# ieellee/uLLSAM

Measured on AMD Instinct MI355X. Metric: images/s end-to-end (ViT+LLM+mask) 1024^2, higher is better.
Workload: dtype bf16; 1 GPU; uLLSAM mask path (app.py:580-645): SAM ViT-H + InternLM2-7b-shaped prefill S=1081 + prompt encoder + mask decoder + x4 upsample/threshold, 1 point prompt/image, batch 4/GPU; batch_per_gpu=4, global_batch=4, seq_len=1081, vit_linears=bf16

## Files before the change

### include/ullsam_hip.h

```cpp
#ifndef ULLSAM_HIP_H
#define ULLSAM_HIP_H
#ifdef __cplusplus
extern "C" {
#endif

#define ULLSAM_DT_F32 0
#define ULLSAM_DT_BF16 1
#define ULLSAM_ACT_NONE 0
#define ULLSAM_ACT_GELU 1
#define ULLSAM_ACT_RELU 2
#define ULLSAM_ACT_SWIGLU 3

#define ULLSAM_ABI_VERSION 14

const char* ullsam_last_error_string(void);
int ullsam_abi_version(void);
int ullsam_device_count(void);
int ullsam_set_gemm_variant(int variant);
int ullsam_set_gemm_tuning(int key, int value);
int ullsam_set_attn_variant(int variant);
int ullsam_set_attn_debug(void* stamps);

#define ULLSAM_ACT_SPLITK_OK 256
int ullsam_gemm(int dtype, const void* A, long lda, const void* W, long ldw, void* C, long ldc, int out_f32,
                const float* bias, const float* residual, long ldr, int res_row_mod, int act, int M, int N, int K,
                void* workspace, long ws_bytes, void* stream);

int ullsam_gemm_qkv_rope(int dtype, const void* A, long lda, const void* W, long ldw, const float* bias, int B, int S, int K, int KVH,
                         int G, const int* pos, const float* cos_tab, const float* sin_tab, int tab_rows, void* q_out, void* k_cache,
                         void* v_cache, int cap, int cache_pos0, void* workspace, long ws_bytes, void* stream);

int ullsam_gemm_panels(int dtype, const void* A, long lda, const void* W, long ldw, const void* w_panels, void* C, long ldc, int out_f32,
                       const float* bias, const float* residual, long ldr, int res_row_mod, int act, int M, int N, int K,
                       void* workspace, long ws_bytes, void* stream);
int ullsam_gemm_qkv_rope_panels(int dtype, const void* A, long lda, const void* W, long ldw, const void* w_panels, const float* bias, int B, int S,
                                int K, int KVH, int G, const int* pos, const float* cos_tab, const float* sin_tab, int tab_rows, void* q_out,
                                void* k_cache, void* v_cache, int cap, int cache_pos0, void* workspace, long ws_bytes, void* stream);

int ullsam_gemm_act_panels(int dtype, const void* A, long lda, const void* W, long ldw, const void* w_panels, void* C, long ldc, int out_f32,
                           const float* bias, const float* residual, long ldr, int res_row_mod, int act, int M, int N, int K,
                           void* workspace, long ws_bytes, int a_panels, int out_panels, void* stream);
int ullsam_gemm_qkv_rope_act_panels(int dtype, const void* A, long lda, const void* W, long ldw, const void* w_panels, const float* bias, int B, int S,
                                    int K, int KVH, int G, const int* pos, const float* cos_tab, const float* sin_tab, int tab_rows, void* q_out,
                                    void* k_cache, void* v_cache, int cap, int cache_pos0, void* workspace, long ws_bytes, int a_panels, void* stream);
int ullsam_gemm_act_panels_query(int dtype, int M, int N, int K, int act, int out_f32, int has_bias, int has_residual, int aligned, long ws_bytes,
                                 int* reads_a_panels, int* writes_c_panels);

int ullsam_gemm_rmsnorm(const float* x, long ldx, const float* norm_w, float eps, const void* W, long ldw, void* C, long ldc, int out_f32,
                        const float* bias, const float* residual, long ldr, int act, int M, int N, int K, void* stream);
int ullsam_decode_qkv_rope(const void* a, const float* x, long ldx, const float* norm_w, float eps, const void* W, long ldw, const float* bias,
                           int B, int K, int KVH, int G, const int* pos, const float* cos_tab, const float* sin_tab, int tab_rows, void* q_out,
                           void* k_cache, void* v_cache, int cap, int cache_pos0, void* stream);

int ullsam_train_matmul(const float* A, const float* B, float* C, int M, int N, int K, int batch, long a_b, long a_m, long a_k, long b_b,
                        long b_k, long b_n, long c_b, long c_m, long c_n, int accumulate, void* stream);
int ullsam_train_matmul_bf16(const float* A, const float* B, float* C, int M, int N, int K, int batch, long a_b, long a_m, long a_k, long b_b,
                             long b_k, long b_n, long c_b, long c_m, long c_n, int accumulate, void* stream);
int ullsam_train_matmul_heads(const float* A, const float* B, float* C, int M, int N, int K, int outer, int heads, long a_o, long a_h, int a_hdiv, long a_m, long a_k,
                              long b_o, long b_h, int b_hdiv, long b_k, long b_n, long c_o, long c_h, long c_m, long c_n, int accumulate, int bf16, int tri, void* stream);
int ullsam_train_matmul_splitk(const float* A, const float* B, float* C, int M, int N, int K, int batch, long a_b, long a_m, long a_k, long b_b,
                               long b_k, long b_n, long c_b, long c_m, long c_n, int accumulate, int ksplit, float* partial, void* stream);
int ullsam_train_set_matmul_mfma(int on);
int ullsam_train_set_matmul_vec(int on);
int ullsam_train_colsum(const float* x, float* out, long rows, int cols, long ld, float* partial, void* stream);
int ullsam_train_ln_bwd(const float* x, const float* w, const float* dy, float* dx, float* dw, float* db, long rows, int D, float eps, float* ws, void* stream);
int ullsam_train_act(const float* x, const float* dy, float* out, long n, int kind, void* stream);
int ullsam_train_scale_shift(const float* x, const float* s, const float* t, const float* dy, float* out, float* ds, float* dt, long n, float* partial, void* stream);
int ullsam_train_attention(const float* q, const float* k, const float* v, const float* dout, float* out, float* dq, float* dk, float* dv,
                           int B, int H, int groups, int hd, int Sq, int Sk, int causal, const int* key_mask, long q_bs, long q_ts, long q_hs,
                           long k_bs, long k_ts, long k_hs, long v_bs, long v_ts, long v_hs, long o_bs, long o_ts, long o_hs, float scale,
                           const float* bias_h, const float* bias_w, float* dbias_h, float* dbias_w, int kw, void* stream);
int ullsam_train_col2im3x3(const float* dcols, float* dx, int B, int H, int W, int C, void* stream);
int ullsam_train_attn_rows(float* S, float* dP, const float* bias_h, const float* bias_w, float* dbias_h, float* dbias_w, const int* key_mask,
                           int B, int H, int Sq, int Sk, int kw, int causal, int have_p, void* stream);
int ullsam_train_set_rows_reg(int on);
int ullsam_train_rmsnorm_bwd(const float* x, const float* w, const float* dy, float* dx, float* dw_rows, long rows, int D, float eps, void* stream);
int ullsam_train_rope(const float* x, const int* pos, const float* cos_tab, const float* sin_tab, float* out, long tokens, int heads, int hd,
                      int tab_rows, int adjoint, void* stream);
int ullsam_train_swiglu(const float* g, const float* u, const float* dy, float* out, float* dg, float* du, long n, void* stream);
int ullsam_train_resize_bwd(const float* dout, float* din, long planes, int ih, int iw, int oh, int ow, void* stream);
int ullsam_train_seg_loss(const float* x, const float* t, float* sums, float* losses, int P, long npix, float smooth, float* partial, void* stream);
int ullsam_train_seg_loss_bwd(const float* x, const float* t, const float* sums, const float* gscale, float* dx, int P, long npix, float smooth, void* stream);
int ullsam_train_cross_entropy(const float* logits, long ld, const long long* labels, float* lse, float* loss_rows, float* out2, long rows, int V, void* stream);
int ullsam_train_cross_entropy_bwd(const float* logits, long ld, const long long* labels, const float* lse, const float* out2, const float* gscale, float* dlogits,
                                   long ldx, long rows, int V, void* stream);
int ullsam_train_cross_entropy_bwd_bf16(const float* logits, long ld, const long long* labels, const float* lse, const float* out2, const float* gscale,
                                        void* dlog, long ldd, void* dlogT, long ldt, long rows, int V, void* stream);
int ullsam_train_embedding_bwd(const float* dx, long ldx, const int* sorted_ids, const int* order, const int* skip, long rows, int D, int V, int padding_idx,
                               void* table_grad, int out_dtype, void* stream);
int ullsam_train_index_add_rows(const float* src, const int* idx, float* dst, long rows, int C, int nrows_dst, void* stream);

int ullsam_norm(const void* in, int in_dtype, long in_stride, void* out, int out_dtype, long out_stride, const float* w,
                const float* b, long rows, int D, float eps, int rms, int act, const float* post_scale,
                const float* post_shift, void* stream);
int ullsam_norm_panels(const void* in, int in_dtype, long in_stride, void* out, const float* w, const float* b, long rows, int D, float eps, int rms,
                       int act, const float* post_scale, const float* post_shift, int out_panels, void* stream);
int ullsam_set_norm_variant(int v);

int ullsam_norm_fanout(const float* in, long rows, int D, const float* w, const float* b, float eps, float* out_f32, void* out_c,
                       void* out_c_pe, int c_dtype, const float* pe, long pe_rows, void* stream);

int ullsam_vit_attention(int dtype, const void* qkv, void* out, const void* rel_h, const void* rel_w, const void* qkv_bias,
                         int B, int heads, int hd, int grid_h, int grid_w, int window, void* stream);

int ullsam_causal_attention(int dtype, const void* q, const void* k, const void* v, void* out, const int* key_mask, int B,
                            int H, int KVH, int hd, int Sq, int Sk, int k_cap, int q_pos0, void* stream);

int ullsam_naive_attention(int dtype, const void* q, const void* k, const void* v, void* out, const int* key_mask, int B,
                           int H, int KVH, int hd, int Sq, int Sk, long q_bs, long q_ts, long q_hs, long k_bs, long k_ts,
                           long k_hs, long v_bs, long v_ts, long v_hs, long o_bs, long o_ts, long o_hs, float scale,
                           void* stream);

int ullsam_decode_attention(const void* q, const void* kc, const void* vc, const int* key_mask, void* out, int B, int H, int KVH,
                            int hd, int Sk, int cap, float scale, float* workspace, int nsplit, void* stream);

int ullsam_fewkeys_attention(const float* q, const float* k, const float* v, float* out, int B, int H, int hd, int Sq,
                             int Sk, float scale, long q_batch_stride, void* stream);

int ullsam_tok2img_attention(int kv_dtype, const float* q, const void* k, const void* v, float* out, int P, int H, int hd, int T,
                             int N, long k_batch_stride, long v_batch_stride, float scale, float* workspace, int nsplit,
                             void* stream);

int ullsam_patch_im2col(int dtype, const float* pixels, void* out, int B, int C, int Hs, int Ws, int S, int patch,
                        const float* mean, const float* stdv, void* stream);
int ullsam_im2col3x3(int dtype, const void* in, void* out, int B, int H, int W, int C, void* stream);
int ullsam_add_cast(const void* a, int a_dtype, long a_rows, const float* b, long b_rows, void* out, int out_dtype,
                    long rows, int cols, void* stream);
int ullsam_transpose_f32(const float* in, float* out, int B, int R, int C, void* stream);
int ullsam_transpose_to_bf16(int in_dtype, const void* in, void* out, int R, int C, int Rp, void* stream);
int ullsam_cast_transpose_bf16(const float* in, void* out_rm, void* out_t, float* colsum_out, float* colsum_ws, int R, int C, int Rp, void* stream);
int ullsam_pixel_shuffle_ln(int dtype, const float* in_nhwc, void* out, const float* w, const float* b, int B, int H, int W,
                            int C, float eps, void* stream);
int ullsam_pixel_unshuffle(const float* in, float* out_nhwc, int B, int H, int W, int C, void* stream);

int ullsam_scan_image_tokens(const long long* ids, int* rank, int* range, int B, int S, long long img_id, void* stream);
int ullsam_embed_tokens(int dtype, const void* table, const long long* ids, const int* rank, const float* vit_embeds,
                        float* out, int B, int S, int D, int n_img, long vocab, void* stream);
int ullsam_gather_rows(const void* in, void* out, const int* range, int B, int S, int n, int row_bytes, void* stream);
int ullsam_rope_split(int dtype, const void* qkv, void* q_out, void* k_cache, void* v_cache, const int* pos,
                      const float* cos_tab, const float* sin_tab, int B, int S, int KVH, int G, int hd, int cap,
                      int cache_pos0, int tab_rows, void* stream);
int ullsam_argmax(const float* logits, long long* out, int rows, long V, long ld, void* stream);
int ullsam_sample_topk_topp(const float* logits, long long* out, int rows, long V, long ld, float temperature, int top_k, float top_p,
                            const unsigned long long* seeds , unsigned long long step,
                            const float* u_in , float* u_out ,
                            long long* cand_ids , float* cand_p , void* stream);

int ullsam_small_linear(const float* x, long ldx, const float* W, const float* b, const float* res, long ldr, float* y,
                        long ldy, int M, int N, int K, int act, void* stream);
int ullsam_i2t_block(const void* xin, long in_mod, const float* res, long res_mod, const void* Wq, const float* bq, const float* ktok,
                     const float* vtok, const void* Wo, const float* bo, const float* lnw, const float* lnb, float eps, const float* key_pe,
                     long pe_rows, float* out_f32, void* out_c, void* out_c_pe, int P, int T, int N, float scale, void* stream);

int ullsam_kv_proj(const void* xk, const void* xv, const void* Wk, const void* Wv, const float* bk, const float* bv, void* K, void* V, long rows, void* stream);
int ullsam_dec_tok_attn(const float* queries, const float* qpe, float* queries_out, float* q_t2i, const void* Wq, const float* bq, const void* Wk, const float* bk,
                        const void* Wv, const float* bv, const void* Wo, const float* bo, const float* ln_w, const float* ln_b, float eps, const void* Wq2,
                        const float* bq2, int P, int T, int skip_pe, int mode, void* stream);
int ullsam_dec_tok_mlp(const float* queries, const float* attn, const float* qpe, float* queries_out, float* k_out, float* v_out, const void* Wo, const float* bo,
                       const float* ln2_w, const float* ln2_b, float eps2, const void* W1, const float* b1, const void* W2, const float* b2, const float* ln3_w,
                       const float* ln3_b, float eps3, const void* Wk, const float* bk, const void* Wv, const float* bv, int P, int T, int do_mlp, void* stream);
int ullsam_dec_heads(const float* hs, const void* const* w, const float* const* b, float* hyper, float* iou, int P, int T, int n_iou, int m0, int nm, void* stream);
int ullsam_concat_token_rows(const float* prefix, int n0, const float* rows, int n1, float* out, int P, int C, void* stream);
int ullsam_up2_hyper_masks(const void* u1, const void* w1, const float* b1, const float* hyper, float* out, int NB, int NM, int H, int W, void* stream);
int ullsam_up1_ln_gelu(const void* src, const void* w0, const float* b0, const float* lnw, const float* lnb, float eps, void* out, long rows, void* stream);
int ullsam_skinny_linear(const float* x, long ldx, const float* WT, const float* b, const float* res, long ldr, float* y,
                         long ldy, int M, int N, int K, int act, void* stream);
int ullsam_set_skinny_linear_mfma(int on);
int ullsam_sparse_embed(const float* coords, const int* labels, const float* boxes, const float* G, const float* emb,
                        float* out, int P, int Np, int pad, int C, float img_w, float img_h, void* stream);
int ullsam_dense_pe(const float* G, float* out_nhwc, int H, int W, int C, void* stream);
int ullsam_mask_downscale(const float* masks, float* out_nhwc, int P, int H, int W, int C, int c1, int c2, const float* w0,
                          const float* b0, const float* g1, const float* be1, const float* w3, const float* b3,
// ... 177 lines not shown
```

### ullsam_amd/_lib.py

```python
from __future__ import annotations

import ctypes as C
import os

_HERE = os.path.dirname(os.path.abspath(__file__))
LIB_PATH = os.environ.get("ULLSAM_HIP_LIB") or os.path.join(_HERE, "lib", "libullsam_hip.so")

ABI_VERSION = 14

_lib = None

vp, i32, i64, f32, f64 = C.c_void_p, C.c_int, C.c_long, C.c_float, C.c_double

SIGNATURES = {
    "ullsam_gemm": [i32, vp, i64, vp, i64, vp, i64, i32, vp, vp, i64, i32, i32, i32, i32, i32, vp, i64, vp],
    "ullsam_gemm_qkv_rope": [i32, vp, i64, vp, i64, vp, i32, i32, i32, i32, i32, vp, vp, vp, i32, vp, vp, vp, i32, i32, vp, i64, vp],
    "ullsam_gemm_panels": [i32, vp, i64, vp, i64, vp, vp, i64, i32, vp, vp, i64, i32, i32, i32, i32, i32, vp, i64, vp],
    "ullsam_gemm_qkv_rope_panels": [i32, vp, i64, vp, i64, vp, vp, i32, i32, i32, i32, i32, vp, vp, vp, i32, vp, vp, vp, i32, i32, vp, i64, vp],
    "ullsam_gemm_act_panels": [i32, vp, i64, vp, i64, vp, vp, i64, i32, vp, vp, i64, i32, i32, i32, i32, i32, vp, i64, i32, i32, vp],
    "ullsam_gemm_qkv_rope_act_panels": [i32, vp, i64, vp, i64, vp, vp, i32, i32, i32, i32, i32, vp, vp, vp, i32, vp, vp, vp, i32, i32, vp, i64, i32, vp],
    "ullsam_gemm_act_panels_query": [i32, i32, i32, i32, i32, i32, i32, i32, i32, i64, vp, vp],
    "ullsam_gemm_rmsnorm": [vp, i64, vp, f32, vp, i64, vp, i64, i32, vp, vp, i64, i32, i32, i32, i32, vp],
    "ullsam_decode_qkv_rope": [vp, vp, i64, vp, f32, vp, i64, vp, i32, i32, i32, i32, vp, vp, vp, i32, vp, vp, vp, i32, i32, vp],
    "ullsam_train_matmul": [vp, vp, vp, i32, i32, i32, i32] + [i64] * 9 + [i32, vp],
    "ullsam_train_matmul_bf16": [vp, vp, vp, i32, i32, i32, i32] + [i64] * 9 + [i32, vp],
    "ullsam_train_matmul_splitk": [vp, vp, vp, i32, i32, i32, i32] + [i64] * 9 + [i32, i32, vp, vp],
    "ullsam_train_matmul_heads": [vp, vp, vp, i32, i32, i32, i32, i32, i64, i64, i32, i64, i64, i64, i64, i32, i64, i64, i64, i64, i64, i64, i32, i32, i32, vp],
    "ullsam_train_colsum": [vp, vp, i64, i32, i64, vp, vp],
    "ullsam_train_ln_bwd": [vp, vp, vp, vp, vp, vp, i64, i32, f32, vp, vp],
    "ullsam_train_act": [vp, vp, vp, i64, i32, vp],
    "ullsam_train_scale_shift": [vp, vp, vp, vp, vp, vp, vp, i64, vp, vp],
    "ullsam_train_attention": [vp] * 8 + [i32] * 7 + [vp] + [i64] * 12 + [f32, vp, vp, vp, vp, i32, vp],
    "ullsam_train_col2im3x3": [vp, vp, i32, i32, i32, i32, vp],
    "ullsam_train_attn_rows": [vp, vp, vp, vp, vp, vp, vp, i32, i32, i32, i32, i32, i32, i32, vp],
    "ullsam_train_rmsnorm_bwd": [vp, vp, vp, vp, vp, i64, i32, f32, vp],
    "ullsam_train_rope": [vp, vp, vp, vp, vp, i64, i32, i32, i32, i32, vp],
    "ullsam_train_swiglu": [vp, vp, vp, vp, vp, vp, i64, vp],
    "ullsam_train_resize_bwd": [vp, vp, i64, i32, i32, i32, i32, vp],
    "ullsam_train_seg_loss": [vp, vp, vp, vp, i32, i64, f32, vp, vp],
    "ullsam_train_seg_loss_bwd": [vp, vp, vp, vp, vp, i32, i64, f32, vp],
    "ullsam_train_cross_entropy": [vp, i64, vp, vp, vp, vp, i64, i32, vp],
    "ullsam_train_cross_entropy_bwd": [vp, i64, vp, vp, vp, vp, vp, i64, i64, i32, vp],
    "ullsam_train_cross_entropy_bwd_bf16": [vp, i64, vp, vp, vp, vp, vp, i64, vp, i64, i64, i32, vp],
    "ullsam_train_embedding_bwd": [vp, i64, vp, vp, vp, i64, i32, i32, i32, vp, i32, vp],
    "ullsam_train_index_add_rows": [vp, vp, vp, i64, i32, i32, vp],
    "ullsam_norm": [vp, i32, i64, vp, i32, i64, vp, vp, i64, i32, f32, i32, i32, vp, vp, vp],
    "ullsam_norm_panels": [vp, i32, i64, vp, vp, vp, i64, i32, f32, i32, i32, vp, vp, i32, vp],
    "ullsam_norm_fanout": [vp, i64, i32, vp, vp, f32, vp, vp, vp, i32, vp, i64, vp],
    "ullsam_vit_attention": [i32, vp, vp, vp, vp, vp, i32, i32, i32, i32, i32, i32, vp],
    "ullsam_causal_attention": [i32, vp, vp, vp, vp, vp, i32, i32, i32, i32, i32, i32, i32, i32, vp],
    "ullsam_naive_attention": [i32, vp, vp, vp, vp, vp, i32, i32, i32, i32, i32, i32] + [i64] * 12 + [f32, vp],
    "ullsam_fewkeys_attention": [vp, vp, vp, vp, i32, i32, i32, i32, i32, f32, i64, vp],
    "ullsam_decode_attention": [vp, vp, vp, vp, vp, i32, i32, i32, i32, i32, i32, f32, vp, i32, vp],
    "ullsam_tok2img_attention": [i32, vp, vp, vp, vp, i32, i32, i32, i32, i32, i64, i64, f32, vp, i32, vp],
    "ullsam_patch_im2col": [i32, vp, vp, i32, i32, i32, i32, i32, i32, vp, vp, vp],
    "ullsam_im2col3x3": [i32, vp, vp, i32, i32, i32, i32, vp],
    "ullsam_add_cast": [vp, i32, i64, vp, i64, vp, i32, i64, i32, vp],
    "ullsam_transpose_f32": [vp, vp, i32, i32, i32, vp],
    "ullsam_transpose_to_bf16": [i32, vp, vp, i32, i32, i32, vp],
    "ullsam_cast_transpose_bf16": [vp, vp, vp, vp, vp, i32, i32, i32, vp],
    "ullsam_pixel_shuffle_ln": [i32, vp, vp, vp, vp, i32, i32, i32, i32, f32, vp],
    "ullsam_pixel_unshuffle": [vp, vp, i32, i32, i32, i32, vp],
    "ullsam_scan_image_tokens": [vp, vp, vp, i32, i32, C.c_longlong, vp],
    "ullsam_embed_tokens": [i32, vp, vp, vp, vp, vp, i32, i32, i32, i32, i64, vp],
    "ullsam_gather_rows": [vp, vp, vp, i32, i32, i32, i32, vp],
    "ullsam_rope_split": [i32, vp, vp, vp, vp, vp, vp, vp, i32, i32, i32, i32, i32, i32, i32, i32, vp],
    "ullsam_argmax": [vp, vp, i32, i64, i64, vp],
    "ullsam_sample_topk_topp": [vp, vp, i32, i64, i64, f32, i32, f32, vp, C.c_ulonglong, vp, vp, vp, vp, vp],
    "ullsam_small_linear": [vp, i64, vp, vp, vp, i64, vp, i64, i32, i32, i32, i32, vp],
    "ullsam_i2t_block": [vp, i64, vp, i64, vp, vp, vp, vp, vp, vp, vp, vp, f32, vp, i64, vp, vp, vp, i32, i32, i32, f32, vp],
    "ullsam_kv_proj": [vp, vp, vp, vp, vp, vp, vp, vp, i64, vp],
    "ullsam_up2_hyper_masks": [vp, vp, vp, vp, vp, i32, i32, i32, i32, vp],
    "ullsam_dec_tok_attn": [vp] * 14 + [f32, vp, vp, i32, i32, i32, i32, vp],
    "ullsam_dec_tok_mlp": [vp] * 10 + [f32] + [vp] * 6 + [f32] + [vp] * 4 + [i32, i32, i32, vp],
    "ullsam_dec_heads": [vp, vp, vp, vp, vp, i32, i32, i32, i32, i32, vp],
    "ullsam_concat_token_rows": [vp, i32, vp, i32, vp, i32, i32, vp],
    "ullsam_up1_ln_gelu": [vp, vp, vp, vp, vp, f32, vp, i64, vp],
    "ullsam_skinny_linear": [vp, i64, vp, vp, vp, i64, vp, i64, i32, i32, i32, i32, vp],
    "ullsam_sparse_embed": [vp, vp, vp, vp, vp, vp, i32, i32, i32, i32, f32, f32, vp],
    "ullsam_dense_pe": [vp, vp, i32, i32, i32, vp],
    "ullsam_mask_downscale": [vp, vp, i32, i32, i32, i32, i32, i32] + [vp] * 10 + [vp],
    "ullsam_hyper_masks": [i32, vp, vp, vp, i32, i32, i32, i32, i32, vp],
    "ullsam_resize_bilinear": [vp, i64, i32, i32, i32, vp, vp, i32, i32, i32, f32, vp],
    "ullsam_mask_iou_counts": [vp, vp, vp, i32, i64, vp],
    "ullsam_stability_score": [vp, i64, i64, f64, f64, vp, vp, vp],
    "ullsam_mask_to_box": [vp, i64, i32, i32, vp, vp],
    "ullsam_rle_pack": [vp, i64, i32, i32, vp, vp, vp, vp],
    "ullsam_rle_emit": [vp, vp, i64, i32, i32, vp, vp, vp],
    "ullsam_amg_postprocess": [vp, vp, i64] + [i32] * 11 + [f64, f64, vp, vp, vp, vp, vp, vp],
    "ullsam_nms_mask": [vp, i32, f32, vp, vp],
    "ullsam_threshold_u8": [vp, vp, i64, f32, vp],
    "ullsam_rle_to_mask": [vp, vp, i64, i32, i32, vp, vp, vp],
    "ullsam_label_regions": [vp, i64, i32, i32, i32, vp, vp],
    "ullsam_remove_small_regions": [vp, vp, i64, i32, i32, i32, i32, vp, i64, vp, vp],
    "ullsam_rle_paint_labels": [vp, vp, vp, i64, i32, i32, vp, vp, vp],
    "ullsam_label_stats": [vp, i64, i32, i32, vp, vp, vp],
    "ullsam_label_compact": [vp, vp, vp, i64, i32, vp, vp, vp, vp, vp, vp],
    "ullsam_label_remap": [vp, vp, i64, i32, i32, vp, vp],
    "ullsam_label_overlap": [vp, vp, i32, i32, i32, i32, vp, vp, vp],
    "ullsam_resize_nearest_i32": [vp, i64, i32, i32, i32, i32, i32, i32, i32, i32, vp, i64, vp],
    "ullsam_mosaic_seams": [vp, i32, i32, i32, vp, i64, vp, i32, i32, vp, vp, i64, i32, vp, vp, vp],
    "ullsam_mosaic_union": [vp, vp, i64, vp, i64, i64, i64, vp, vp, vp],
    "ullsam_mosaic_stats": [vp, i32, i32, i32, vp, i64, vp, i32, vp, i32, i32, vp, vp, vp, vp],
    "ullsam_mosaic_compact": [vp, vp, vp, i64, i32, vp, vp, vp, vp, vp],
    "ullsam_mosaic_paste": [vp, i32, i32, i32, vp, i64, vp, i32, vp, i32, i32, vp, vp],
    "ullsam_stack_pairs": [vp, i32, i32, i32, vp, i64, vp, vp, i64, i32, vp, vp, vp],
    "ullsam_stack_best": [vp, vp, i64, vp, i64, i64, i64, vp, vp, vp, vp],
    "ullsam_stack_link": [vp, vp, vp, vp, i64, vp, i64, i64, i64, vp, vp, vp],
    "ullsam_stack_stats": [vp, i32, i32, i32, vp, i64, vp, vp, vp, vp, vp, vp],
    "ullsam_stack_compact": [vp, vp, vp, vp, i64, i32, i64, vp, vp, vp, vp, vp, vp],
    "ullsam_stack_relabel": [vp, i32, i32, i32, vp, i64, vp, vp, vp],
    "ullsam_distance_columns": [vp, i32, i32, i32, i32, i64, vp, vp, vp, vp],
    "ullsam_distance_rows": [vp, vp, vp, i32, i32, i32, i32, i64, i32, i64, vp, vp, vp, vp, vp],
    "ullsam_distance_depth_decode": [vp, i64, i32, vp, vp, vp],
    "ullsam_distance3d_z": [vp, i32, i32, i32, i32, i32, i64, vp, vp, vp, vp],
    "ullsam_distance3d_y": [vp, vp, vp, i32, i32, i32, i32, i32, i32, i32, i32, i32, i32, i64, vp, vp, vp],
    "ullsam_distance3d_x": [vp, vp, vp, i32, i32, i32, i32, i32, i32, i32, i32, i32, i32, i64, i64, vp, vp, vp, vp, vp],
    "ullsam_distance3d_depth_decode": [vp, i64, i32, i32, vp, vp, vp],
    "ullsam_split_ascent": [vp, vp, i32, i32, i64, i32, vp, vp, vp],
    "ullsam_split_flatten": [vp, i64, i64, vp, vp],
    "ullsam_split_passes": [vp, vp, vp, i32, i32, i64, vp, vp, i64, i32, vp, vp],
    "ullsam_split_round": [vp, vp, i64, vp, vp, i64, i64, i32, vp, vp, vp, vp, vp],
    "ullsam_split_collect": [vp, vp, i64, i64, vp, i64, vp, vp],
    "ullsam_split_relabel": [vp, i64, vp, vp, vp, i32, i32, i64, vp, vp, vp, vp, vp, vp, vp, vp],
    "ullsam_split3d_ascent": [vp, vp, i32, i32, i32, i64, i32, vp, vp, vp],
    "ullsam_split3d_passes": [vp, vp, vp, i32, i32, i32, i64, vp, vp, i64, i32, vp, vp],
    "ullsam_split3d_relabel": [vp, i64, vp, vp, vp, i32, i32, i32, i64, vp, vp, vp, vp, vp, vp, vp, vp],
    "ullsam_outline_sides": [vp, i32, i32, i64, vp, vp, vp, vp, vp],
    "ullsam_outline_scan": [vp, i64, vp, vp, vp, vp],
    "ullsam_outline_successors": [vp, i32, i32, vp, vp, i64, i32, vp, vp, vp, vp, vp],
    "ullsam_outline_rank": [vp, vp, vp, i64, i32, vp, vp, vp, vp, vp],
    "ullsam_outline_collect": [vp, i64, vp, vp, i64, vp, i64, vp, vp],
    "ullsam_outline_loops": [vp, vp, vp, i64, i64, i32, vp, vp, vp, vp],
    "ullsam_outline_order": [vp, vp, vp, vp, vp, vp, i64, i64, vp, vp, vp, vp],
    "ullsam_outline_vertices": [vp, vp, vp, i64, i32, i64, vp, vp],
    "ullsam_outline_parents": [vp, i32, i32, vp, vp, vp, vp, vp, vp, vp, i64, i64, vp, vp, vp],
    "ullsam_simplify_flags": [vp, i32, i32, vp, vp, i64, vp, vp, vp],
    "ullsam_simplify_candidates": [vp, vp, vp, vp, i64, i64, i64, i32, i32, vp, vp, vp, vp, vp, vp],
    "ullsam_simplify_anchors": [vp, vp, vp, i64, i64, vp, vp, vp, vp],
    "ullsam_simplify_segments": [vp, vp, vp, vp, vp, i64, i64, vp, vp, vp, vp, vp],
    "ullsam_simplify_rounds": [vp, vp, vp, i64, i64, C.c_longlong, i32, vp, vp, vp, vp, vp, vp, vp],
    "ullsam_simplify_rings": [vp, vp, vp, vp, vp, vp, i64, i64, i64, vp, vp, vp, vp, vp, vp],
    "ullsam_raster_scan": [vp, i64, vp, vp, vp, vp, vp],
    "ullsam_raster_edges": [vp, i64, vp, i64, vp, i32, i32, i64, vp, vp, vp, vp, vp, vp, vp, vp],
    "ullsam_raster_keys": [vp, i64, vp, vp, vp, vp, vp, i64, i32, i32, i64, vp, vp, vp],
    "ullsam_raster_covered": [vp, i64, i32, i32, i64, vp, vp, vp, vp],
    "ullsam_raster_paint": [vp, i64, vp, i32, i32, i64, i32, vp, vp, vp, vp, vp],
    "ullsam_raster_finish": [vp, i32, i32, vp, i64, vp, vp, vp, vp, vp],
    "ullsam_measure_instances": [vp, i32, i32, i32, vp, i32, i32, i32, vp, vp, vp, vp, vp, vp, vp, vp, vp, vp],
    "ullsam_label_contacts": [vp, i32, i32, i32, vp, vp, i64, i32, vp, vp, vp],
    "ullsam_measure_objects3d": [vp, i32, i32, i32, i32, vp, i32, i32, i32, vp, vp, vp, vp, vp, vp, vp, vp, vp, vp],
    "ullsam_object_contacts3d": [vp, i32, i32, i32, i32, vp, vp, i64, i32, vp, vp, vp],
    "ullsam_label_d1": [vp, i32, i32, i32, vp, vp, vp, vp],
    "ullsam_prompt_choose": [vp, i32, C.c_ulonglong, vp, vp, vp, vp, vp],
    "ullsam_prompt_sets": [vp, vp, i32, i32, vp, vp, vp, vp, i32, i32, i32, i32, vp, vp, vp, vp, vp, vp],
    "ullsam_prompt_points": [i32, i32, vp, vp, vp, vp, i32, i32, i32, i32, C.c_ulonglong, vp, vp, vp, vp, vp, vp, vp],
    "ullsam_instance_masks": [vp, vp, i64, i64, vp, vp],
    "ullsam_resize_u8_aa_h": [vp, i64, i64, i64, i32, i32, i32, i32, i32, i32, i32, i32, i32, vp, vp, i32, i32, vp, vp],
    "ullsam_resize_u8_aa_v": [vp, i32, i32, i32, i32, vp, vp, i32, i32, vp, vp, vp, i64, i64, vp],
    "ullsam_minmax_u16": [vp, i64, vp, vp],
    "ullsam_minmax_f32": [vp, i64, vp, vp],
    "ullsam_normalize_to_u8_u16": [vp, i64, vp, vp, vp],
    "ullsam_normalize_to_u8_f32": [vp, i64, vp, vp, vp],
    "ullsam_click_finish": [vp] + [i32] * 9 + [f32, vp, vp, i32, i32, vp, i32, vp, vp, vp, vp, vp, vp],
    "ullsam_rows_fp8": [vp, i32, i64, vp, i64, vp, vp, vp, i64, i32, f32, vp],
    "ullsam_gemm_fp8": [vp, i64, vp, vp, i64, vp, vp, i64, i32, vp, vp, i64, i32, i32, i32, i32, vp],
    "ullsam_rows_fp8_pow2": [vp, i32, i64, vp, i64, vp, i64, i32, vp],
    "ullsam_gemm_w8": [vp, vp, i64, vp, f32, vp, i64, vp, vp, i64, i32, vp, vp, i64, i32, i32, i32, i32, vp],
    "ullsam_decode_qkv_rope_w8": [vp, vp, i64, vp, f32, vp, i64, vp, vp, i32, i32, i32, i32, vp, vp, vp, i32, vp, vp, vp, i32, i32, vp],
}
PLAIN = {"ullsam_last_error_string": ([], C.c_char_p), "ullsam_abi_version": ([], i32), "ullsam_device_count": ([], i32),
         "ullsam_set_gemm_variant": ([i32], i32), "ullsam_set_gemm_tuning": ([i32, i32], i32), "ullsam_set_attn_variant": ([i32], i32),
         "ullsam_set_norm_variant": ([i32], i32), "ullsam_train_set_matmul_mfma": ([i32], i32), "ullsam_train_set_matmul_vec": ([i32], i32), "ullsam_train_set_rows_reg": ([i32], i32), "ullsam_set_skinny_linear_mfma": ([i32], i32), "ullsam_set_attn_debug": ([vp], i32)}


class UllsamError(RuntimeError):
    pass


def load():
    global _lib
    if _lib is not None:
        return _lib
    if not os.path.exists(LIB_PATH):
        raise UllsamError(f"{LIB_PATH} not found -- run `python -m ullsam_amd.build` (there is no CPU fallback)")
    import torch
    lib = C.CDLL(LIB_PATH)
    for name, args in SIGNATURES.items():
        fn = getattr(lib, name)
        fn.argtypes = args
        fn.restype = i32
    for name, (args, res) in PLAIN.items():
        fn = getattr(lib, name)
        fn.argtypes = args
        fn.restype = res
    got = lib.ullsam_abi_version()
    if got != ABI_VERSION:
        raise UllsamError(f"{LIB_PATH} reports ABI version {got}, this binding is version {ABI_VERSION}: stale build -- run `python -m ullsam_amd.build --force`")
    _lib = lib
    return lib


def call(name: str, *args):
    lib = load()
    rc = getattr(lib, name)(*args)
    if rc != 0:
        msg = lib.ullsam_last_error_string()
        raise UllsamError(f"{name} failed ({rc}): {msg.decode() if msg else '?'}")
```

### ullsam_amd/csrc/gemm.hip

```cpp
#include "common.h"
#include <type_traits>

struct GemmArgs {
    const void* A;
    const void* W;
    void* C;
    const float* bias;
    const float* residual;
    int M, N, K;
    long lda, ldw, ldc, ldr;
    int res_row_mod;
    int act;
    int out_f32;
    int vec_ok;
    int tiles_m, tiles_n;
    int full_tiles, ksplit;
    float* ws;
    size_t ws_bytes;
    const int* rope_pos; const float* rope_cos; const float* rope_sin; void* rope_q; void* rope_k; void* rope_v;
    int rope_S, rope_KVH, rope_G, rope_cap, rope_pos0, rope_rows;
    const float* row_scale;
    const float* col_scale;
    unsigned long long* dbg;
    const float* norm_x; const float* norm_w; float norm_eps; long ldx;
    const void* w_panels;
    int group_m;
    int a_panels, out_panels;
    int* plan;
};

#ifndef ULLSAM_RING_ASM_DMA
#define ULLSAM_RING_ASM_DMA 1
#endif
static constexpr bool g_asm_dma = ULLSAM_RING_ASM_DMA != 0;
static int g_split_tail = 1;
static int g_gemm_variant = 0;
static int g_dbg = 0;
static int g_auto_mask = 7;
static int g_group_m = 4;

template <typename T>
__device__ __forceinline__ Frag<T> lds_frag(const char* tile, int row, int ks, int g);
template <>
__device__ __forceinline__ Frag<bf16> lds_frag<bf16>(const char* tile, int row, int ks, int g) {
    const int c = (ks * 4 + g) ^ (row & 7);
    return load_frag(reinterpret_cast<const bf16*>(tile + row * 128 + (c << 4)));
}
template <>
__device__ __forceinline__ Frag<float> lds_frag<float>(const char* tile, int row, int ks, int g) {
    (void)ks;
    const int c0 = (2 * g) ^ (row & 7), c1 = (2 * g + 1) ^ (row & 7);
    const float4 a = *reinterpret_cast<const float4*>(tile + row * 128 + (c0 << 4));
    const float4 b = *reinterpret_cast<const float4*>(tile + row * 128 + (c1 << 4));
    Frag<float> f;
    f.v[0] = a.x; f.v[1] = a.y; f.v[2] = a.z; f.v[3] = a.w;
    f.v[4] = b.x; f.v[5] = b.y; f.v[6] = b.z; f.v[7] = b.w;
    return f;
}

template <typename OutT>
__device__ __forceinline__ void store_row8(OutT* dst, const float* v, int n_valid, bool vec);
template <>
__device__ __forceinline__ void store_row8<float>(float* dst, const float* v, int n_valid, bool vec) {
    if (vec && n_valid == 8) {
        *reinterpret_cast<float4*>(dst) = make_float4(v[0], v[1], v[2], v[3]);
        *reinterpret_cast<float4*>(dst + 4) = make_float4(v[4], v[5], v[6], v[7]);
    } else {
        for (int e = 0; e < n_valid; ++e) dst[e] = v[e];
    }
}
template <>
__device__ __forceinline__ void store_row8<bf16>(bf16* dst, const float* v, int n_valid, bool vec) {
    if (vec && n_valid == 8) {
        bf16x8_t o;
#pragma unroll
        for (int e = 0; e < 8; ++e) o[e] = (bf16)v[e];
        *reinterpret_cast<bf16x8_t*>(dst) = o;
    } else {
        for (int e = 0; e < n_valid; ++e) dst[e] = (bf16)v[e];
    }
}


template <typename T, typename OutT, int BM, int NTHREADS, int BN = 128, int EMODE = 0, bool RING16 = false>
__device__ __forceinline__ void epilogue_rows(const GemmArgs& p, const float* Cs, int m0, int n0, int tn, int tid) {
    constexpr int TPR = BN / 8;
    constexpr int RPP = NTHREADS / TPR;
    constexpr int PASSES = (BM + RPP - 1) / RPP;
    constexpr bool RAGGED = BM % RPP != 0;
    static_assert(NTHREADS % TPR == 0, "threads per pass must cover whole rows");
    if (RAGGED && tid >= NTHREADS) return;
    OutT* C = reinterpret_cast<OutT*>(p.C);
    if (p.act == 3) {
#pragma unroll
        for (int pass = 0; pass < PASSES; ++pass) {
            const int row = pass * RPP + tid / TPR;
            const int t = tid % TPR;
            const int grp = t >> 4, j0 = (t & 15) * 4;
            const int gm = m0 + row;
            if (gm >= p.M) continue;
            const float4 g = *reinterpret_cast<const float4*>(Cs + row * BN + grp * 128 + j0);
            const float4 u = *reinterpret_cast<const float4*>(Cs + row * BN + grp * 128 + 64 + j0);
            float4 o;
            if constexpr (RING16) {
                o = make_float4(g.x * __builtin_amdgcn_rcpf(1.0f + __expf(-g.x)) * u.x, g.y * __builtin_amdgcn_rcpf(1.0f + __expf(-g.y)) * u.y,
                                g.z * __builtin_amdgcn_rcpf(1.0f + __expf(-g.z)) * u.z, g.w * __builtin_amdgcn_rcpf(1.0f + __expf(-g.w)) * u.w);
            } else {
                o = make_float4(silu_f(g.x) * u.x, silu_f(g.y) * u.y, silu_f(g.z) * u.z, silu_f(g.w) * u.w);
            }
            OutT* dst = C + (size_t)gm * p.ldc + (size_t)tn * (BN / 2) + grp * 64 + j0;
            if (p.vec_ok) {
                store4(dst, o);
            } else {
                dst[0] = from_f32<OutT>(o.x); dst[1] = from_f32<OutT>(o.y);
                dst[2] = from_f32<OutT>(o.z); dst[3] = from_f32<OutT>(o.w);
            }
        }
        return;
    }
    if constexpr (EMODE == 1) {
        const int c0 = (tid % TPR) * 8;
        const int gn = n0 + c0;
        if (gn >= p.N) return;
        const int slot = gn >> 7, d = gn & 127;
        const int gs = p.rope_G + 2, kv = slot / gs, g = slot - kv * gs;
        const int pc = d < 64 ? c0 + 64 : c0 - 64;
        float bx[8], bp[8];
#pragma unroll
        for (int e = 0; e < 8; ++e) { bx[e] = p.bias ? p.bias[gn + e] : 0.f; bp[e] = p.bias ? p.bias[gn + (pc - c0) + e] : 0.f; }
        T* Q = reinterpret_cast<T*>(p.rope_q);
        T* Kc = reinterpret_cast<T*>(p.rope_k);
        T* Vc = reinterpret_cast<T*>(p.rope_v);
        const bool rotate = g != gs - 1;
        int ps[PASSES];
#pragma unroll
        for (int pass = 0; pass < PASSES; ++pass) {
            const int gm = m0 + pass * RPP + tid / TPR;
            ps[pass] = (rotate && gm < p.M) ? min(max(p.rope_pos[gm], 0), p.rope_rows - 1) : 0;
        }
        float4 cn[2], sn[2];
        auto load_cs = [&](int pass, float4 (&c)[2], float4 (&s_)[2]) {
            const float* cp = p.rope_cos + (size_t)ps[pass] * 128 + d;
            const float* sp = p.rope_sin + (size_t)ps[pass] * 128 + d;
            c[0] = *reinterpret_cast<const float4*>(cp); c[1] = *reinterpret_cast<const float4*>(cp + 4);
            s_[0] = *reinterpret_cast<const float4*>(sp); s_[1] = *reinterpret_cast<const float4*>(sp + 4);
        };
        if (rotate) load_cs(0, cn, sn);
#pragma unroll
        for (int pass = 0; pass < PASSES; ++pass) {
            const int row = pass * RPP + tid / TPR;
            const int gm = m0 + row;
            float4 cc[2] = {cn[0], cn[1]}, ss[2] = {sn[0], sn[1]};
            if (rotate && pass + 1 < PASSES) load_cs(pass + 1, cn, sn);
            if (gm >= p.M) continue;
            float x[8], y[8], o[8];
            const float4 xa = *reinterpret_cast<const float4*>(Cs + row * BN + c0), xb = *reinterpret_cast<const float4*>(Cs + row * BN + c0 + 4);
            const float4 ya = *reinterpret_cast<const float4*>(Cs + row * BN + pc), yb = *reinterpret_cast<const float4*>(Cs + row * BN + pc + 4);
            x[0] = xa.x; x[1] = xa.y; x[2] = xa.z; x[3] = xa.w; x[4] = xb.x; x[5] = xb.y; x[6] = xb.z; x[7] = xb.w;
            y[0] = ya.x; y[1] = ya.y; y[2] = ya.z; y[3] = ya.w; y[4] = yb.x; y[5] = yb.y; y[6] = yb.z; y[7] = yb.w;
#pragma unroll
            for (int e = 0; e < 8; ++e) { x[e] += bx[e]; y[e] += bp[e]; }
            const int b = gm / p.rope_S, sq = gm - b * p.rope_S;
            if (!rotate) {
#pragma unroll
                for (int e = 0; e < 8; ++e) o[e] = x[e];
            } else {
                const float cv[8] = {cc[0].x, cc[0].y, cc[0].z, cc[0].w, cc[1].x, cc[1].y, cc[1].z, cc[1].w};
                const float sv[8] = {ss[0].x, ss[0].y, ss[0].z, ss[0].w, ss[1].x, ss[1].y, ss[1].z, ss[1].w};
#pragma unroll
                for (int e = 0; e < 8; ++e) o[e] = d < 64 ? x[e] * cv[e] - y[e] * sv[e] : x[e] * cv[e] + y[e] * sv[e];
            }
            T* dst;
            if (g < p.rope_G) dst = Q + (size_t)gm * ((size_t)p.rope_KVH * p.rope_G * 128) + (size_t)(kv * p.rope_G + g) * 128 + d;
            else dst = (g == gs - 2 ? Kc : Vc) + (((size_t)b * p.rope_KVH + kv) * p.rope_cap + p.rope_pos0 + sq) * 128 + d;
            store_row8<T>(dst, o, 8, true);
        }
        return;
    }
    const int c0 = (tid % TPR) * 8;
    const int gn = n0 + c0;
    if (gn >= p.N) return;
    const int n_valid = min(8, p.N - gn);
    float bv[8];
#pragma unroll
    for (int e = 0; e < 8; ++e) bv[e] = 0.f;
    if (p.bias) {
        if (n_valid == 8 && ((reinterpret_cast<uintptr_t>(p.bias + gn) & 15) == 0)) {
            const float4 b0 = *reinterpret_cast<const float4*>(p.bias + gn);
            const float4 b1 = *reinterpret_cast<const float4*>(p.bias + gn + 4);
            bv[0] = b0.x; bv[1] = b0.y; bv[2] = b0.z; bv[3] = b0.w; bv[4] = b1.x; bv[5] = b1.y; bv[6] = b1.z; bv[7] = b1.w;
        } else {
// ... 305 lines not shown
            for (int ks = 0; ks < KSTEPS; ++ks) {
                Frag<T> b[4], a8[8];
#pragma unroll
                for (int j = 0; j < 4; ++j) b[j] = lds_frag<T>(Bb, wn * 64 + j * 16 + (lane & 15), ks, lane >> 4);
#pragma unroll
                for (int i = 0; i < 8; ++i) a8[i] = lds_frag<T>(Ab, wm * 128 + i * 16 + (lane & 15), ks, lane >> 4);
                __builtin_amdgcn_s_setprio(1);
#pragma unroll
                for (int i = 0; i < 8; ++i)
#pragma unroll
                    for (int j = 0; j < 4; ++j) mma16(a8[i], b[j], acc[i][j]);
                __builtin_amdgcn_s_setprio(0);
            }
        }
    }

    float* Cs = reinterpret_cast<float*>(smem);
#pragma unroll
    for (int half = 0; half < 2; ++half) {
        __syncthreads();
        if (wm == half) {
#pragma unroll
            for (int i = 0; i < 8; ++i)
#pragma unroll
                for (int j = 0; j < 4; ++j)
#pragma unroll
                    for (int r = 0; r < 4; ++r) {
                        const int row = i * 16 + 4 * (lane >> 4) + r;
                        const int col = wn * 64 + j * 16 + (lane & 15);
                        Cs[row * 256 + col] = acc[i][j][r];
                    }
        }
        __syncthreads();
        if (part >= 0) {
            float4* dst = reinterpret_cast<float4*>(p.ws + ((size_t)tail_idx * p.ksplit + part) * 65536 + half * 32768);
            const float4* src = reinterpret_cast<const float4*>(Cs);
#pragma unroll
            for (int i = 0; i < 16; ++i) dst[i * 512 + tid] = src[i * 512 + tid];
        } else if (p.out_f32) {
            epilogue_rows<T, float, 128, 512, 256, EMODE>(p, Cs, m0 + half * 128, n0, tn, tid);
        } else {
            epilogue_rows<T, T, 128, 512, 256, EMODE>(p, Cs, m0 + half * 128, n0, tn, tid);
        }
    }
}

template <typename T, int ROWS, int NT, int EMODE = 0>
__global__ __launch_bounds__(NT) void gemm256_tail_reduce_kernel(GemmArgs p) {
    __shared__ __attribute__((aligned(16))) float Cs[ROWS * 256];
    constexpr int SPT = 256 / ROWS;
    constexpr int VPT = ROWS * 64 / NT;
    const int tid = threadIdx.x;
    const int tail_idx = blockIdx.x / SPT, slab = blockIdx.x % SPT;
    const int swz = p.full_tiles + tail_idx;
    const int GM = p.group_m;
    const int width = GM * p.tiles_n;
    const int group = swz / width;
    const int first_m = group * GM;
    const int gsize = min(p.tiles_m - first_m, GM);
    const int tm = first_m + (swz % width) % gsize;
    const int tn = (swz % width) / gsize;
    const float4* src = reinterpret_cast<const float4*>(p.ws + (size_t)tail_idx * p.ksplit * 65536 + slab * (ROWS * 256));
    float4 acc[VPT];
#pragma unroll
    for (int i = 0; i < VPT; ++i) acc[i] = make_float4(0.f, 0.f, 0.f, 0.f);
#pragma unroll 8
    for (int s = 0; s < p.ksplit; ++s) {
#pragma unroll
        for (int i = 0; i < VPT; ++i) {
            const float4 b = src[(size_t)s * 16384 + i * NT + tid];
            acc[i].x += b.x; acc[i].y += b.y; acc[i].z += b.z; acc[i].w += b.w;
        }
    }
#pragma unroll
    for (int i = 0; i < VPT; ++i) reinterpret_cast<float4*>(Cs)[i * NT + tid] = acc[i];
    __syncthreads();
    const int mrow = tm * 256 + slab * ROWS;
    if (p.out_f32)
        epilogue_rows<T, float, ROWS, NT, 256, EMODE>(p, Cs, mrow, tn * 256, tn, tid);
    else
        epilogue_rows<T, T, ROWS, NT, 256, EMODE>(p, Cs, mrow, tn * 256, tn, tid);
}

typedef __attribute__((ext_vector_type(4))) unsigned int u32x4;
typedef __attribute__((ext_vector_type(2))) unsigned int u32x2;

__device__ __forceinline__ void gstore16(void* ptr, u32x4 v) {
    *reinterpret_cast<u32x4*>(ptr) = v;
}
__device__ __forceinline__ unsigned int pack_bf16x2(float lo, float hi) {
    typedef __attribute__((ext_vector_type(2))) __bf16 bf16x2_t;
    bf16x2_t v;
    v[0] = (bf16)lo; v[1] = (bf16)hi;
    return __builtin_bit_cast(unsigned int, v);
}

__device__ __forceinline__ unsigned int lane_xor1(unsigned int v) {
    return (unsigned int)__builtin_amdgcn_mov_dpp((int)v, 0xB1, 0xF, 0xF, true);
}
__device__ __forceinline__ void pair_swap(const u32x4& lo, const u32x4& hi, bool odd, u32x4& first, u32x4& second) {
    u32x4 send, recv;
#pragma unroll
    for (int e = 0; e < 4; ++e) send[e] = odd ? lo[e] : hi[e];
#pragma unroll
    for (int e = 0; e < 4; ++e) recv[e] = lane_xor1(send[e]);
#pragma unroll
    for (int e = 0; e < 4; ++e) { first[e] = odd ? recv[e] : lo[e]; second[e] = odd ? hi[e] : recv[e]; }
}

template <typename T, int EMODE = 0>
static int launch_gemm_v3_impl(GemmArgs a, hipStream_t stream) {
    static PerDeviceOnce attr_set;
    if (attr_set.first()) {
        (void)hipFuncSetAttribute(reinterpret_cast<const void*>(gemm256_kernel<T, EMODE>), hipFuncAttributeMaxDynamicSharedMemorySize, 131072);
    }
    a.tiles_m = (a.M + 255) / 256;
    a.tiles_n = (a.N + 255) / 256;
    const int T_ = a.tiles_m * a.tiles_n;
    const int nk = a.K / (128 / (int)sizeof(T));
    const int tail = T_ % 256;
    a.full_tiles = T_;
    a.ksplit = 1;
    if (g_split_tail && a.ws && T_ > 256 && tail > 0 && tail <= 64 && nk >= 64) {
        int S = 256 / tail;
        if (S > 8) S = 8;
        if (S > nk / 8) S = nk / 8;
        if (S >= 2 && (size_t)tail * S * 262144 <= a.ws_bytes) {
            a.full_tiles = T_ - tail;
            a.ksplit = S;
        }
    }
    gemm256_kernel<T, EMODE><<<dim3(a.full_tiles + (T_ - a.full_tiles) * a.ksplit), dim3(512), 131072, stream>>>(a);
    ULLSAM_LAUNCH_CHECK();
    if (a.ksplit > 1) {
        const int tail_tiles = T_ - a.full_tiles;
        if (tail_tiles * a.ksplit <= 128) gemm256_tail_reduce_kernel<T, 4, 128, EMODE><<<dim3(tail_tiles * 64), dim3(128), 0, stream>>>(a);
        else gemm256_tail_reduce_kernel<T, 16, 256, EMODE><<<dim3(tail_tiles * 16), dim3(256), 0, stream>>>(a);
        ULLSAM_LAUNCH_CHECK();
    }
    return 0;
}
template <typename T>
static int launch_gemm_v3(GemmArgs a, hipStream_t stream) {
    if (a.act == 4) return launch_gemm_v3_impl<T, 1>(a, stream);
    return launch_gemm_v3_impl<T, 0>(a, stream);
}

__device__ __forceinline__ void glds16_sbase(const char* base, unsigned int off, unsigned int lds_addr) {
    unsigned int keep;
    asm volatile("s_mov_b32 %0, m0\n\ts_mov_b32 m0, %3\n\ts_nop 0\n\tglobal_load_lds_dwordx4 %1, %2\n\ts_mov_b32 m0, %0"
                 : "=&s"(keep) : "v"(off), "s"(base), "s"(lds_addr) : "memory");
}

template <int MI0, int MI1, int NTW, bool STAMP = false, int EMODE = 0>
__global__ __launch_bounds__(512) void gemm_ring8_kernel(GemmArgs p) {
    extern __shared__ __attribute__((aligned(16))) char smem[];
    const unsigned long long t_entry = STAMP ? __builtin_amdgcn_s_memtime() : 0ull;
    typedef bf16 T;
    constexpr int BM = 16 * (MI0 + MI1), BN = 64 * NTW, MI = MI0 > MI1 ? MI0 : MI1;
    constexpr int PA = BM / 16, PB = BN / 16;
    constexpr int ASZ = BM * 64, STG = ASZ + BN * 64;
    static_assert(PA >= 8 && PA <= 24 && PB >= 8 && PB <= 24, "piece assignment below: one to three pieces per wave and operand");
    if constexpr (EMODE == 2) {
        p.K /= (int)gridDim.y;
        p.A = reinterpret_cast<const char*>(p.A) + (size_t)blockIdx.y * p.K * 2;
        p.W = reinterpret_cast<const char*>(p.W) + (size_t)blockIdx.y * p.K * 2;
        p.C = reinterpret_cast<float*>(p.C) + (size_t)blockIdx.y * p.M * p.ldc;
    }

    const int nblk = p.full_tiles;
    const int bid = blockIdx.x;
    const int q8 = nblk >> 3, r8 = nblk & 7, xcd = bid & 7;
    const int swz = (xcd < r8 ? xcd * (q8 + 1) : r8 * (q8 + 1) + (xcd - r8) * q8) + (bid >> 3);
    const int GM = p.group_m;
    const int width = GM * p.tiles_n;
    const int group = swz / width;
    const int first_m = group * GM;
    const int gsize = min(p.tiles_m - first_m, GM);
    const int tm = first_m + (swz % width) % gsize;
    const int tn = (swz % width) / gsize;
    const int m0 = tm * BM, n0 = tn * BN;

    const int tid = threadIdx.x, lane = tid & 63;
    const int wave = __builtin_amdgcn_readfirstlane(tid >> 6);
    const int wm = wave >> 2, wn = wave & 3, grp = wave >> 2;
    const int g4 = lane >> 4, mm = lane & 15;

    const char* a_base = reinterpret_cast<const char*>(p.A) + (size_t)m0 * p.lda * 2;
    const bool panels = EMODE != 2 && p.w_panels != nullptr;
    const unsigned int kst = __builtin_amdgcn_readfirstlane(panels ? 1024u : 64u);
    const char* b_base = reinterpret_cast<const char*>(panels ? p.w_panels : p.W) + (size_t)n0 * p.ldw * 2;
    const bool a_pan = EMODE != 2 && p.a_panels != 0;
    const unsigned int akst = __builtin_amdgcn_readfirstlane(a_pan ? 1024u : 64u);
    const int na = (PA - wave + 7) / 8, nb = (PB - wave + 7) / 8;
    static_assert(NTW == 4 || NTW == 5, "epilogue layouts below: four sub-tiles in two pairs, optionally a fifth on its own");
    constexpr int WW = 16 * NTW;
    const int perm = EMODE == 1 ? 2 : p.out_f32 ? 0 : (p.act == 3 ? 2 : 1);
    auto w_row = [&](int R) {
        const int wb = R / WW, q = R - wb * WW, j = q >> 4, r = q & 15;
        if (perm == 1) return j < 4 ? WW * wb + 32 * (j >> 1) + 8 * (r >> 2) + 4 * (j & 1) + (r & 3) : WW * wb + 64 + r;
        if (perm == 2) return 128 * (wb >> 1) + 64 * (j >> 1) + 32 * (wb & 1) + 8 * (r >> 2) + 4 * (j & 1) + (r & 3);
        return R;
    };
    unsigned int a_off[3], b_off[3];
#pragma unroll
    for (int i = 0; i < 3; ++i) {
        const int row = (wave + 8 * i) * 16 + (lane >> 2);
        const int c = (lane & 3) ^ ((row >> 2) & 2);
        if (a_pan) {
            const int ar = min(m0 + row, ((p.M + 15) & ~15) - 1) - m0;
            a_off[i] = (unsigned int)(ar >> 4) * ((unsigned int)p.K * 32u) + (unsigned int)(ar & 15) * 64u + (c << 4);
        } else {
            a_off[i] = (unsigned int)((size_t)(min(m0 + row, p.M - 1) - m0) * p.lda * 2) + (c << 4);
        }
        const int wr = w_row(row);
        b_off[i] = panels ? (unsigned int)(wr >> 4) * ((unsigned int)p.K * 32u) + (unsigned int)(wr & 15) * 64u + (c << 4)
                          : (unsigned int)((size_t)(min(n0 + wr, p.N - 1) - n0) * p.ldw * 2) + (c << 4);
    }
    const int st1 = p.K >> 5;

    const int mi = wm == 0 ? MI0 : MI1;
    const int row_w = wm == 0 ? 0 : MI0 * 16;
    f32x4 acc[MI][NTW];
#pragma unroll
    for (int i = 0; i < MI; ++i)
#pragma unroll
        for (int j = 0; j < NTW; ++j) acc[i][j] = (f32x4){0.f, 0.f, 0.f, 0.f};

    auto stage = [&](int s) {
        char* base = smem + (s & 3) * STG;
        const char* ak = a_base + (size_t)s * akst;
        const char* bk = b_base + (size_t)s * kst;
#pragma unroll
        for (int i = 0; i < 3; ++i) {
            if (i < na) __builtin_amdgcn_global_load_lds(GLB_PTR(ak + a_off[i]), LDS_PTR(base + (wave + 8 * i) * 1024), 16, 0, 0);
            if (i < nb) __builtin_amdgcn_global_load_lds(GLB_PTR(bk + b_off[i]), LDS_PTR(base + ASZ + (wave + 8 * i) * 1024), 16, 0, 0);
        }
    };
    auto frag = [&](const char* tile, int row) -> Frag<T> {
        return load_frag(reinterpret_cast<const T*>(tile + row * 64 + ((g4 ^ ((row >> 2) & 2)) << 4)));
    };
    const int npc = na + nb;
    auto wait_one_left = [&]() {
        if (npc == 4) asm volatile("s_waitcnt vmcnt(4)" ::: "memory");
        else if (npc == 2) asm volatile("s_waitcnt vmcnt(2)" ::: "memory");
        else if (npc == 5) asm volatile("s_waitcnt vmcnt(5)" ::: "memory");
        else if (npc == 6) asm volatile("s_waitcnt vmcnt(6)" ::: "memory");
        else asm volatile("s_waitcnt vmcnt(3)" ::: "memory");
    };

    const bool has_bias = p.bias && p.act != 3 && EMODE == 0;
    char* const bias_lds = smem + (st1 & 3) * STG;
    auto bias_dma = [&]() __attribute__((always_inline)) {
        if (has_bias && wave < (BN * 4 + 1023) / 1024) {
            const int c = min(n0 + wave * 256 + lane * 4, p.N - 4);
            __builtin_amdgcn_global_load_lds(GLB_PTR(p.bias + c), LDS_PTR(bias_lds + wave * 1024), 16, 0, 0);
        }
    };
    stage(0);
    if (1 < st1) { stage(1); wait_one_left(); }
    else asm volatile("s_waitcnt vmcnt(0)" ::: "memory");
    __builtin_amdgcn_s_barrier();
    if (grp == 1) __builtin_amdgcn_s_barrier();
    auto stamp = [&](int kk) {
        if (STAMP && p.dbg && (tid & 255) == 0) p.dbg[((size_t)bid * 2 + grp) * 4 + kk] = __builtin_amdgcn_s_memtime();
    };
    auto stamp16 = [&](int kk) {
        if (STAMP && p.dbg && (tid & 255) == 0) p.dbg[(1 << 19) + ((size_t)bid * 2 + grp) * 8 + kk] = __builtin_amdgcn_s_memtime();
    };
    stamp(0);
    {
        auto body = [&](int s, auto NA_c, auto NB_c, auto MORE_c) __attribute__((always_inline)) {
            constexpr int NA = decltype(NA_c)::value, NB = decltype(NB_c)::value;
            constexpr bool MORE = decltype(MORE_c)::value;
            const char* Ab = smem + (s & 3) * STG;
            const char* Bb = Ab + ASZ;
            Frag<T> a8[MI], b[NTW];
            {
                char* base = smem + ((s + 2) & 3) * STG;
                const char* ak = a_base + (size_t)(s + 2) * akst;
                const char* bk = b_base + (size_t)(s + 2) * kst;
                auto request = [&](int qi) __attribute__((always_inline)) {
                    const int i = qi >> 1;
                    if (g_asm_dma) {
                        if (MORE && !(qi & 1) && i < NA) glds16_sbase(ak, a_off[i], (unsigned int)(uintptr_t)LDS_PTR(base + (wave + 8 * i) * 1024));
                        if (MORE && (qi & 1) && i < NB) glds16_sbase(bk, b_off[i], (unsigned int)(uintptr_t)LDS_PTR(base + ASZ + (wave + 8 * i) * 1024));
                    } else {
                        if (MORE && !(qi & 1) && i < NA) __builtin_amdgcn_global_load_lds(GLB_PTR(ak + a_off[i]), LDS_PTR(base + (wave + 8 * i) * 1024), 16, 0, 0);
                        if (MORE && (qi & 1) && i < NB) __builtin_amdgcn_global_load_lds(GLB_PTR(bk + b_off[i]), LDS_PTR(base + ASZ + (wave + 8 * i) * 1024), 16, 0, 0);
                    }
                    __builtin_amdgcn_sched_barrier(0);
                };
                int qi = 0;
                request(qi++);
#pragma unroll
                for (int r = 0; r < NTW + MI; ++r) {
                    if (r < NTW) b[r] = frag(Bb, wn * (16 * NTW) + r * 16 + mm);
                    else if ((r - NTW) < MI1 || (r - NTW) < mi) a8[r - NTW] = frag(Ab, row_w + (r - NTW) * 16 + mm);
                    __builtin_amdgcn_sched_barrier(0);
                    if ((r % 3) == 2 && qi < 6) request(qi++);
                }
#pragma unroll
                for (; qi < 6; ++qi) request(qi);
            }
            if constexpr (!MORE) asm volatile("s_waitcnt vmcnt(0)" ::: "memory");
            else if constexpr (NA + NB == 4) asm volatile("s_waitcnt vmcnt(4)" ::: "memory");
            else if constexpr (NA + NB == 5) asm volatile("s_waitcnt vmcnt(5)" ::: "memory");
            else if constexpr (NA + NB == 6) asm volatile("s_waitcnt vmcnt(6)" ::: "memory");
            else if constexpr (NA + NB == 3) asm volatile("s_waitcnt vmcnt(3)" ::: "memory");
            else asm volatile("s_waitcnt vmcnt(2)" ::: "memory");
            __builtin_amdgcn_sched_barrier(0);
            __builtin_amdgcn_s_barrier();
            __builtin_amdgcn_s_setprio(1);
#pragma unroll
            for (int i = 0; i < MI; ++i)
                if (i < MI1 || i < mi) {
#pragma unroll
                    for (int j = 0; j < NTW; ++j) mma16(b[j], a8[i], acc[i][j]);
                }
            __builtin_amdgcn_s_setprio(0);
            __builtin_amdgcn_sched_barrier(0);
            __builtin_amdgcn_s_barrier();
        };
        auto run = [&](auto NA_c, auto NB_c) __attribute__((always_inline)) {
            int s = 0;
            for (; s + 2 < st1; ++s) body(s, NA_c, NB_c, std::true_type{});
            bias_dma();
            for (; s < st1; ++s) body(s, NA_c, NB_c, std::false_type{});
        };
        constexpr int NA_LO = PA / 8, NA_HI = (PA + 7) / 8, NB_LO = PB / 8, NB_HI = (PB + 7) / 8;
        if (NA_HI != NA_LO && na == NA_HI) {
            if (NB_HI != NB_LO && nb == NB_HI) run(std::integral_constant<int, NA_HI>{}, std::integral_constant<int, NB_HI>{});
            else run(std::integral_constant<int, NA_HI>{}, std::integral_constant<int, NB_LO>{});
        } else {
            if (NB_HI != NB_LO && nb == NB_HI) run(std::integral_constant<int, NA_LO>{}, std::integral_constant<int, NB_HI>{});
            else run(std::integral_constant<int, NA_LO>{}, std::integral_constant<int, NB_LO>{});
        }
    }
    if (grp == 0) __builtin_amdgcn_s_barrier();
    stamp(1);
    float bv[4 * NTW];
#pragma unroll
    for (int e = 0; e < 4 * NTW; ++e) bv[e] = 0.f;
    if (has_bias) {
#pragma unroll
        for (int t = 0; t < NTW; ++t) {
            const int col = wn * WW + ((p.out_f32 || t == 4) ? 16 * t + 4 * g4 : 32 * (t >> 1) + 8 * g4 + 4 * (t & 1));
            const float4 x = *reinterpret_cast<const float4*>(bias_lds + col * 4);
            bv[4 * t] = x.x; bv[4 * t + 1] = x.y; bv[4 * t + 2] = x.z; bv[4 * t + 3] = x.w;
        }
    }

    {
        const bool odd = mm & 1;
        const int row0 = m0 + row_w + mm;
        const int rowp = row0 & ~1;
        const bool direct = p.vec_ok && (p.N & 7) == 0 && (p.M & 1) == 0 && (p.out_f32 || !p.residual);
        auto gst = [&](void* ptr, u32x4 v) __attribute__((always_inline)) { *reinterpret_cast<u32x4*>(ptr) = v; };
        const bool o_pan = p.out_panels != 0;
        const size_t o_cells = (size_t)((p.act == 3 ? p.N >> 1 : p.N) >> 5);
        const size_t o_r16 = o_pan ? o_cells * 512 : (size_t)16 * p.ldc, o_r1 = o_pan ? (size_t)32 : (size_t)p.ldc;
        auto o_at = [&](int row, int col) __attribute__((always_inline)) -> size_t {
            return o_pan ? ((size_t)(row >> 4) * o_cells + (size_t)(col >> 5)) * 512 + (size_t)((row & 15) * 32 + (col & 31)) : (size_t)row * p.ldc + col;
        };
        if constexpr (EMODE == 1) {
            const int slot = (n0 >> 7) + (wn >> 1), d = 32 * (wn & 1) + 8 * g4;
            const int gs = p.rope_G + 2, kv = slot / gs, g = slot - kv * gs;
            const bool live = slot < p.rope_KVH * gs;
            const bool rotate = g != gs - 1;
            float bl[8], bh[8];
#pragma unroll
            for (int e = 0; e < 8; ++e) { bl[e] = (p.bias && live) ? p.bias[slot * 128 + d + e] : 0.f; bh[e] = (p.bias && live) ? p.bias[slot * 128 + d + 64 + e] : 0.f; }
            T* const Q = reinterpret_cast<T*>(p.rope_q);
            T* const KVc = reinterpret_cast<T*>(g == gs - 2 ? p.rope_k : p.rope_v);
            int ps[MI];
#pragma unroll
            for (int i = 0; i < MI; ++i) {
                const int gm = row0 + 16 * i;
                ps[i] = (live && rotate && gm < p.M && (i < MI1 || i < mi)) ? min(max(p.rope_pos[gm], 0), p.rope_rows - 1) : 0;
            }
            float4 cn[2], sn[2];
            auto load_cs = [&](int i, float4 (&c)[2], float4 (&s_)[2]) __attribute__((always_inline)) {
                const float* cp = p.rope_cos + (size_t)ps[i] * 128 + d;
                const float* sp = p.rope_sin + (size_t)ps[i] * 128 + d;
                c[0] = *reinterpret_cast<const float4*>(cp); c[1] = *reinterpret_cast<const float4*>(cp + 4);
                s_[0] = *reinterpret_cast<const float4*>(sp); s_[1] = *reinterpret_cast<const float4*>(sp + 4);
            };
            if (rotate) load_cs(0, cn, sn);
#pragma unroll
            for (int i = 0; i < MI; ++i) {
                const float4 c0 = cn[0], c1 = cn[1], s0 = sn[0], s1 = sn[1];
                if (rotate && i + 1 < MI) load_cs(i + 1, cn, sn);
                const int gm = row0 + 16 * i;
                if (!(i < MI1 || i < mi) || gm >= p.M || !live) continue;
                float x[8], y[8], lo[8], hi[8];
#pragma unroll
                for (int e = 0; e < 8; ++e) { x[e] = acc[i][e >> 2][e & 3] + bl[e]; y[e] = acc[i][2 + (e >> 2)][e & 3] + bh[e]; }
                if (rotate) {
                    const float cv[8] = {c0.x, c0.y, c0.z, c0.w, c1.x, c1.y, c1.z, c1.w}, sv[8] = {s0.x, s0.y, s0.z, s0.w, s1.x, s1.y, s1.z, s1.w};
#pragma unroll
                    for (int e = 0; e < 8; ++e) { lo[e] = fmaf(x[e], cv[e], -(y[e] * sv[e])); hi[e] = fmaf(y[e], cv[e], x[e] * sv[e]); }
                } else {
#pragma unroll
                    for (int e = 0; e < 8; ++e) { lo[e] = x[e]; hi[e] = y[e]; }
                }
                T* dst;
                if (g < p.rope_G) dst = Q + (size_t)gm * ((size_t)p.rope_KVH * p.rope_G * 128) + (size_t)(kv * p.rope_G + g) * 128 + d;
                else {
                    const int bi = gm / p.rope_S, sq = gm - bi * p.rope_S;
                    dst = KVc + (((size_t)bi * p.rope_KVH + kv) * p.rope_cap + p.rope_pos0 + sq) * 128 + d;
                }
                gst(dst, (u32x4){pack_bf16x2(lo[0], lo[1]), pack_bf16x2(lo[2], lo[3]), pack_bf16x2(lo[4], lo[5]), pack_bf16x2(lo[6], lo[7])});
                gst(dst + 64, (u32x4){pack_bf16x2(hi[0], hi[1]), pack_bf16x2(hi[2], hi[3]), pack_bf16x2(hi[4], hi[5]), pack_bf16x2(hi[6], hi[7])});
            }
        } else if (direct && !p.out_f32 && p.act != 3) {
            const int colb = n0 + wn * WW + (odd ? 32 : 0) + 8 * g4;
            T* cp = reinterpret_cast<T*>(p.C) + o_at(rowp, colb);
            const int col5 = n0 + wn * WW + 64 + 4 * g4;
            T* cp5 = reinterpret_cast<T*>(p.C) + o_at(row0, col5);
            auto drain = [&](auto ACT) __attribute__((always_inline)) {
                uint2 w5 = make_uint2(0u, 0u);
                auto actf = [&](float v) __attribute__((always_inline)) {
                    if constexpr (decltype(ACT)::value == 1) return gelu_erfc5(v);
                    else if constexpr (decltype(ACT)::value == 2) return fmaxf(v, 0.f);
                    else return v;
                };
#pragma unroll
                for (int i = 0; i < MI; ++i) {
                    if (!(i < MI1 || i < mi)) continue;
                    unsigned int o[8];
#pragma unroll
                    for (int h = 0; h < 2; ++h)
#pragma unroll
                        for (int q = 0; q < 4; ++q)
                            o[4 * h + q] = pack_bf16x2(actf(acc[i][2 * h + (q >> 1)][2 * (q & 1)] + bv[8 * h + 2 * q]),
                                                       actf(acc[i][2 * h + (q >> 1)][2 * (q & 1) + 1] + bv[8 * h + 2 * q + 1]));
                    u32x4 s0, s1;
                    pair_swap((u32x4){o[0], o[1], o[2], o[3]}, (u32x4){o[4], o[5], o[6], o[7]}, odd, s0, s1);
                    if (rowp + 16 * i < p.M && colb < p.N) {
                        gst(cp + i * o_r16, s0);
                        gst(cp + i * o_r16 + o_r1, s1);
                    }
                    if constexpr (NTW == 5) {
                        uint2 w;
                        w.x = pack_bf16x2(actf(acc[i][4][0] + bv[16]), actf(acc[i][4][1] + bv[17]));
                        w.y = pack_bf16x2(actf(acc[i][4][2] + bv[18]), actf(acc[i][4][3] + bv[19]));
                        if constexpr (MI0 == MI1 && MI % 2 == 0) {
                            if (i & 1) {
                                const auto rx = __builtin_amdgcn_permlane16_swap(w5.x, w.x, false, false);
                                const auto ry = __builtin_amdgcn_permlane16_swap(w5.y, w.y, false, false);
                                const int r5 = row0 + 16 * (i - 1 + (g4 & 1));
                                if (r5 < p.M && col5 < p.N)
                                    gst(reinterpret_cast<T*>(p.C) + o_at(r5, n0 + wn * WW + 64 + 8 * (g4 >> 1)), (u32x4){rx[0], ry[0], rx[1], ry[1]});
                            } else {
                                w5 = w;
                            }
                        } else {
                            if (row0 + 16 * i < p.M && col5 < p.N) *reinterpret_cast<uint2*>(cp5 + i * o_r16) = w;
                        }
                    }
                }
            };
            if (p.act == 1) drain(std::integral_constant<int, 1>{});
            else if (p.act == 2) drain(std::integral_constant<int, 2>{});
            else drain(std::integral_constant<int, 0>{});
        } else if (NTW == 4 && direct && !p.out_f32 && p.act == 3) {
            T* cp = reinterpret_cast<T*>(p.C) + o_at(row0, (n0 >> 1) + (wn >> 1) * 64 + (wn & 1) * 32 + 8 * g4);
#pragma unroll
            for (int i = 0; i < MI; ++i) {
                if (!(i < MI1 || i < mi)) continue;
                unsigned int o[4];
#pragma unroll
                for (int q = 0; q < 4; ++q) {
                    const float g0 = acc[i][q >> 1][2 * (q & 1)], g1 = acc[i][q >> 1][2 * (q & 1) + 1];
                    const float u0 = acc[i][2 + (q >> 1)][2 * (q & 1)], u1 = acc[i][2 + (q >> 1)][2 * (q & 1) + 1];
                    o[q] = pack_bf16x2(g0 * __builtin_amdgcn_rcpf(1.0f + __expf(-g0)) * u0, g1 * __builtin_amdgcn_rcpf(1.0f + __expf(-g1)) * u1);
                }
                if (row0 + 16 * i < p.M) gst(cp + i * o_r16, (u32x4){o[0], o[1], o[2], o[3]});
            }
        } else if (direct && p.out_f32 && p.act == 0) {
            const int colp = n0 + wn * WW + (odd ? 16 : 0) + 4 * g4;
            float* cp = reinterpret_cast<float*>(p.C) + (size_t)rowp * p.ldc + colp;
            const int col5 = n0 + wn * WW + 64 + 4 * g4;
            float* cp5 = reinterpret_cast<float*>(p.C) + (size_t)row0 * p.ldc + col5;
            auto load_res = [&](int i, float4 (&r)[5]) __attribute__((always_inline)) {
#pragma unroll
                for (int rsel = 0; rsel < 2; ++rsel) {
                    const int gm = min(rowp + 16 * i + rsel, p.M - 1);
                    const int rr = p.res_row_mod > 0 ? gm % p.res_row_mod : gm;
                    const float* rp = p.residual + (size_t)rr * p.ldr + colp;
#pragma unroll
                    for (int jp = 0; jp < 2; ++jp) r[2 * jp + rsel] = colp + 32 * jp < p.N ? *reinterpret_cast<const float4*>(rp + 32 * jp) : make_float4(0.f, 0.f, 0.f, 0.f);
                }
                if constexpr (NTW == 5) {
                    const int gm = min(row0 + 16 * i, p.M - 1);
                    const int rr = p.res_row_mod > 0 ? gm % p.res_row_mod : gm;
                    r[4] = col5 < p.N ? *reinterpret_cast<const float4*>(p.residual + (size_t)rr * p.ldr + col5) : make_float4(0.f, 0.f, 0.f, 0.f);
                }
            };
            auto put = [&](int i, const float4 (&r)[5]) __attribute__((always_inline)) {
#pragma unroll
                for (int jp = 0; jp < 2; ++jp) {
                    u32x4 lo, hi, s0, s1;
#pragma unroll
                    for (int e = 0; e < 4; ++e) {
                        lo[e] = __float_as_uint(acc[i][2 * jp][e] + bv[8 * jp + e]);
                        hi[e] = __float_as_uint(acc[i][2 * jp + 1][e] + bv[8 * jp + 4 + e]);
                    }
                    pair_swap(lo, hi, odd, s0, s1);
                    const float4 r0 = r[2 * jp], r1 = r[2 * jp + 1];
                    s0 = (u32x4){__float_as_uint(__uint_as_float(s0[0]) + r0.x), __float_as_uint(__uint_as_float(s0[1]) + r0.y),
                                 __float_as_uint(__uint_as_float(s0[2]) + r0.z), __float_as_uint(__uint_as_float(s0[3]) + r0.w)};
                    s1 = (u32x4){__float_as_uint(__uint_as_float(s1[0]) + r1.x), __float_as_uint(__uint_as_float(s1[1]) + r1.y),
                                 __float_as_uint(__uint_as_float(s1[2]) + r1.z), __float_as_uint(__uint_as_float(s1[3]) + r1.w)};
                    if (rowp + 16 * i < p.M && colp + 32 * jp < p.N) {
                        *reinterpret_cast<u32x4*>(cp + (size_t)(16 * i) * p.ldc + 32 * jp) = s0;
                        *reinterpret_cast<u32x4*>(cp + (size_t)(16 * i + 1) * p.ldc + 32 * jp) = s1;
                    }
                }
                if constexpr (NTW == 5) {
                    if (row0 + 16 * i < p.M && col5 < p.N)
                        *reinterpret_cast<float4*>(cp5 + (size_t)(16 * i) * p.ldc) = make_float4(acc[i][4][0] + bv[16] + r[4].x, acc[i][4][1] + bv[17] + r[4].y,
                                                                                                 acc[i][4][2] + bv[18] + r[4].z, acc[i][4][3] + bv[19] + r[4].w);
                }
            };
            auto drain = [&](auto RES) __attribute__((always_inline)) {
                float4 ra[5], rb[5];
#pragma unroll
                for (int j = 0; j < 5; ++j) ra[j] = rb[j] = make_float4(0.f, 0.f, 0.f, 0.f);
                if constexpr (decltype(RES)::value) load_res(0, ra);
#pragma unroll
                for (int i = 0; i < MI; i += 2) {
                    if constexpr (decltype(RES)::value) { if (i + 1 < MI) load_res(i + 1, rb); __builtin_amdgcn_sched_barrier(0); }
                    if (i < MI1 || i < mi) put(i, ra);
                    if constexpr (decltype(RES)::value) { if (i + 2 < MI) load_res(i + 2, ra); __builtin_amdgcn_sched_barrier(0); }
                    if (i + 1 < MI && (i + 1 < MI1 || i + 1 < mi)) put(i + 1, rb);
                }
            };
            if (p.residual) drain(std::true_type{}); else drain(std::false_type{});
        } else {
            float* Cs = reinterpret_cast<float*>(smem);
            auto ncol = [&](int j) __attribute__((always_inline)) {
                if (perm == 1) return j < 4 ? WW * wn + 32 * (j >> 1) + 8 * g4 + 4 * (j & 1) : WW * wn + 64 + 4 * g4;
                if (perm == 2) return 128 * (wn >> 1) + 64 * (j >> 1) + 32 * (wn & 1) + 8 * g4 + 4 * (j & 1);
                return WW * wn + 16 * j + 4 * g4;
            };
            auto staged = [&](auto half_c) __attribute__((always_inline)) {
                constexpr int half = decltype(half_c)::value;
                constexpr int ROWS = 16 * (half == 0 ? MI0 : MI1);
                constexpr int NT_E = (512 / (BN / 8)) * (BN / 8);
                __syncthreads();
                if (wm == half) {
#pragma unroll
                    for (int i = 0; i < (half == 0 ? MI0 : MI1); ++i)
#pragma unroll
                        for (int j = 0; j < NTW; ++j)
                            *reinterpret_cast<float4*>(Cs + (i * 16 + mm) * BN + ncol(j)) = make_float4(acc[i][j][0], acc[i][j][1], acc[i][j][2], acc[i][j][3]);
                }
                __syncthreads();
                if (p.out_f32) epilogue_rows<T, float, ROWS, NT_E, BN>(p, Cs, m0 + half * 16 * MI0, n0, tn, tid);
                else epilogue_rows<T, T, ROWS, NT_E, BN, 0, true>(p, Cs, m0 + half * 16 * MI0, n0, tn, tid);
            };
            staged(std::integral_constant<int, 0>{});
            staged(std::integral_constant<int, 1>{});
        }
    }
    stamp(2);
    if (STAMP && p.dbg && (tid & 255) == 0) p.dbg[((size_t)bid * 2 + grp) * 4 + 3] = t_entry;
}

template <int MI0, int MI1, int NTW, int EMODE = 0>
static int launch_gemm_ring8(GemmArgs a, hipStream_t stream) {
    constexpr int BM = 16 * (MI0 + MI1), BN = 64 * NTW;
    constexpr int LDS = (4 * (BM + BN) * 64 > 16 * MI0 * BN * 4) ? 4 * (BM + BN) * 64 : 16 * MI0 * BN * 4;
    static_assert(LDS <= 163840, "160 KiB of LDS per CU");
    static PerDeviceOnce attr_set;
    if (attr_set.first()) {
        (void)hipFuncSetAttribute(reinterpret_cast<const void*>(gemm_ring8_kernel<MI0, MI1, NTW, false, EMODE>), hipFuncAttributeMaxDynamicSharedMemorySize, LDS);
        if constexpr (EMODE == 0) (void)hipFuncSetAttribute(reinterpret_cast<const void*>(gemm_ring8_kernel<MI0, MI1, NTW, true>), hipFuncAttributeMaxDynamicSharedMemorySize, LDS);
    }
    a.tiles_m = (a.M + BM - 1) / BM;
    a.tiles_n = (a.N + BN - 1) / BN;
    a.full_tiles = a.tiles_m * a.tiles_n;
    a.ksplit = 1;
    if constexpr (EMODE == 0) {
        if (a.dbg) {
            gemm_ring8_kernel<MI0, MI1, NTW, true><<<dim3(a.full_tiles), dim3(512), LDS, stream>>>(a);
            ULLSAM_LAUNCH_CHECK();
            return 0;
        }
    }
    gemm_ring8_kernel<MI0, MI1, NTW, false, EMODE><<<dim3(a.full_tiles), dim3(512), LDS, stream>>>(a);
    ULLSAM_LAUNCH_CHECK();
    return 0;
}
template <typename TO>
__global__ __launch_bounds__(256) void splitk_finish_kernel(const float* __restrict__ ws, TO* __restrict__ C, long ldc, const float* __restrict__ bias,
                                                            const float* __restrict__ residual, long ldr, int res_row_mod, int M, int N, int S) {
    const long q = (long)blockIdx.x * 256 + threadIdx.x, nq = N >> 2;
    if (q >= (long)M * nq) return;
    const int m = (int)(q / nq), c = (int)(q - (long)m * nq) * 4;
    const size_t plane = (size_t)M * N;
    const float* src = ws + (size_t)m * N + c;
    float4 v[8];
#pragma unroll
    for (int k = 0; k < 8; ++k) if (k < S) v[k] = *reinterpret_cast<const float4*>(src + k * plane);
    float4 s = v[0];
#pragma unroll
    for (int k = 1; k < 8; ++k) if (k < S) { s.x += v[k].x; s.y += v[k].y; s.z += v[k].z; s.w += v[k].w; }
    if (bias) { const float4 b = *reinterpret_cast<const float4*>(bias + c); s.x += b.x; s.y += b.y; s.z += b.z; s.w += b.w; }
    if (residual) {
        const int rr = res_row_mod > 0 ? m % res_row_mod : m;
        const float4 r = *reinterpret_cast<const float4*>(residual + (size_t)rr * ldr + c);
        s.x += r.x; s.y += r.y; s.z += r.z; s.w += r.w;
    }
    if constexpr (sizeof(TO) == 4) *reinterpret_cast<float4*>(C + (size_t)m * ldc + c) = s;
    else *reinterpret_cast<uint2*>(C + (size_t)m * ldc + c) = make_uint2(pack_bf16x2(s.x, s.y), pack_bf16x2(s.z, s.w));
}
template <int MI0, int MI1, int NTW>
static int launch_gemm_ring_splitk(const GemmArgs& a, int S, hipStream_t stream) {
    constexpr int BM = 16 * (MI0 + MI1), BN = 64 * NTW;
    constexpr int LDS = (4 * (BM + BN) * 64 > 16 * MI0 * BN * 4) ? 4 * (BM + BN) * 64 : 16 * MI0 * BN * 4;
    static PerDeviceOnce attr_set;
    if (attr_set.first()) (void)hipFuncSetAttribute(reinterpret_cast<const void*>(gemm_ring8_kernel<MI0, MI1, NTW, false, 2>), hipFuncAttributeMaxDynamicSharedMemorySize, LDS);
    GemmArgs b = a;
    b.C = a.ws; b.ldc = a.N; b.out_f32 = 1; b.bias = nullptr; b.residual = nullptr; b.act = 0; b.vec_ok = 1; b.dbg = nullptr; b.w_panels = nullptr; b.a_panels = b.out_panels = 0;
    b.tiles_m = (a.M + BM - 1) / BM;
    b.tiles_n = (a.N + BN - 1) / BN;
    b.full_tiles = b.tiles_m * b.tiles_n;
    b.ksplit = 1;
    gemm_ring8_kernel<MI0, MI1, NTW, false, 2><<<dim3(b.full_tiles, S), dim3(512), LDS, stream>>>(b);
    ULLSAM_LAUNCH_CHECK();
    const long quads = (long)a.M * (a.N >> 2);
    if (a.out_f32) splitk_finish_kernel<float><<<dim3((unsigned)((quads + 255) / 256)), 256, 0, stream>>>(a.ws, static_cast<float*>(a.C), a.ldc, a.bias, a.residual, a.ldr, a.res_row_mod, a.M, a.N, S);
    else splitk_finish_kernel<bf16><<<dim3((unsigned)((quads + 255) / 256)), 256, 0, stream>>>(a.ws, static_cast<bf16*>(a.C), a.ldc, a.bias, a.residual, a.ldr, a.res_row_mod, a.M, a.N, S);
    ULLSAM_LAUNCH_CHECK();
    return 0;
}
static int g_ring_splitk = 1;
static int ring_splitk_plan(const GemmArgs& a, int* shape) {
    if (a.act != 0 || !a.vec_ok || !a.ws || (a.N & 7) != 0 || a.M < 1024 || a.N < 256 || a.dbg) return 0;
    const long t272 = (long)((a.M + 271) / 272) * ((a.N + 255) / 256), t256 = (long)((a.M + 255) / 256) * ((a.N + 255) / 256);
    const long t320 = a.N % 320 == 0 ? (long)((a.M + 255) / 256) * (a.N / 320) : 1l << 40;
    const double a272 = 1.0625 * t272, a256 = 1.0 * t256, a320 = 1.25 * t320;
    long t; if (a320 <= a272 && a320 <= a256) { t = t320; *shape = 8; } else if (a272 < a256) { t = t272; *shape = 9; } else { t = t256; *shape = 6; }
    if (t > 128) return 0;
    int S = (int)(256 / t); if (S > 8) S = 8;
    while (S >= 2 && (a.K % (64 * S) != 0 || a.K / S < 1280 || (size_t)S * a.M * a.N * 4 > a.ws_bytes)) --S;
    return (S >= 2 && S * t >= 224) ? S : 0;
}
#include "gemm_ring8p.h"
static int g_persist = 2;
static int g_ring_panels = 1;
static int g_act_panels = 1;
static int cu_count() {
    static int n[32] = {};
    int d = 0;
    (void)hipGetDevice(&d);
    d &= 31;
    if (!n[d]) { int v = 0; if (hipDeviceGetAttribute(&v, hipDeviceAttributeMultiprocessorCount, d) != hipSuccess || v <= 0) v = 256; n[d] = v; }
    return n[d];
}
template <int BM, int BN, int NTW, int EMODE>
static bool ring_persist_ok(const GemmArgs& a) {
    if (!g_persist || a.N % BN != 0 || a.K % 128 != 0 || a.K < 384 || (a.dbg && !(g_dbg & 2))) return false;
    const long tiles = (long)((a.M + BM - 1) / BM) * (a.N / BN);
    if (tiles <= cu_count()) return false;
    if (((size_t)(a.M + BM) * a.lda + a.K) * 2 >= (1ull << 32) || ((size_t)a.N * a.ldw + a.K) * 2 >= (1ull << 32)) return false;
    if (EMODE == 1) return true;
    if (!(a.vec_ok && (a.N & 7) == 0 && (a.M & 1) == 0)) return false;
    if (!a.out_f32) return !a.residual && (a.act != 3 || NTW == 4);
    return a.act == 0;
}
template <int MI0, int MI1, int NTW, int EMODE = 0>
static int launch_ring(const GemmArgs& a0, hipStream_t stream) {
    GemmArgs a = a0;
    if (!(g_ring_panels && a.N % (64 * NTW) == 0 && a.K % 32 == 0 && a.ldw == a.K)) a.w_panels = nullptr;
    const int n_out = a.act == 3 ? a.N / 2 : a.N;
    const bool a_ok = g_act_panels && EMODE != 2 && a.K % 32 == 0 && a.lda == a.K && ((uintptr_t)a.A & 1023) == 0;
    const bool c_ok = g_act_panels && EMODE == 0 && !a.out_f32 && !a.residual && a.vec_ok && (a.N & 7) == 0 && (a.M & 1) == 0 && (a.act != 3 || NTW == 4) &&
                      n_out % 32 == 0 && a.ldc == n_out && ((uintptr_t)a.C & 1023) == 0;
    if (a.plan) { a.plan[0] = a_ok; a.plan[1] = c_ok; return 0; }
    if ((a.a_panels && !a_ok) || (a.out_panels && !c_ok)) {
        ullsam_set_error("ullsam_gemm: activation K-panels refused (A %d, C %d): this launch reads A as panels %d, can write C as panels %d -- ask the query first", a.a_panels, a.out_panels, (int)a_ok, (int)c_ok);
        return -1;
    }
    return ring_persist_ok<16 * (MI0 + MI1), 64 * NTW, NTW, EMODE>(a) ? launch_gemm_ring8p<MI0, MI1, NTW, EMODE>(a, stream, cu_count())
                                                                      : launch_gemm_ring8<MI0, MI1, NTW, EMODE>(a, stream);
}
static int launch_gemm_v6(const GemmArgs& a, hipStream_t stream) { return launch_ring<8, 8, 4>(a, stream); }
static int launch_gemm_v8(const GemmArgs& a, hipStream_t stream) { return launch_ring<8, 8, 5>(a, stream); }
static int launch_gemm_v9(const GemmArgs& a, hipStream_t stream) { return launch_ring<9, 8, 4>(a, stream); }
static int launch_gemm_ring_rope(const GemmArgs& a, hipStream_t stream, int force) {
    auto cost = [&](int bm) { const long t = (long)((a.M + bm - 1) / bm) * ((a.N + 255) / 256); return (double)((t + 255) / 256) * bm / 256.0; };
    const double c208 = cost(208), c256 = cost(256), c272 = cost(272);
    int pick = (c208 < c256 && c208 < c272) ? 208 : (c272 < c256 ? 272 : 256);
    if (force) pick = force;
    if (pick == 208) return launch_ring<7, 6, 4, 1>(a, stream);
    if (pick == 272) return launch_ring<9, 8, 4, 1>(a, stream);
    return launch_ring<8, 8, 4, 1>(a, stream);
}

typedef __attribute__((ext_vector_type(8))) int i32x8;
__device__ __forceinline__ int f8_swz(int row) { return (row & 6) | ((row >> 3) & 1); }
__device__ __forceinline__ i32x8 lds_frag8(const char* tile, int row, int g) {
    const int f = f8_swz(row);
    const int4 lo = *reinterpret_cast<const int4*>(tile + row * 128 + (((2 * g) ^ f) << 4));
    const int4 hi = *reinterpret_cast<const int4*>(tile + row * 128 + (((2 * g + 1) ^ f) << 4));
    return (i32x8){lo.x, lo.y, lo.z, lo.w, hi.x, hi.y, hi.z, hi.w};
}
__global__ __launch_bounds__(512) void gemm256f8_kernel(GemmArgs p) {
    extern __shared__ __attribute__((aligned(16))) char smem[];
    constexpr int STAGE = 65536;
    const int nblk = p.tiles_m * p.tiles_n;
    const int bid = blockIdx.x;
    const int q8 = nblk >> 3, r8 = nblk & 7, xcd = bid & 7;
    const int swz = (xcd < r8 ? xcd * (q8 + 1) : r8 * (q8 + 1) + (xcd - r8) * q8) + (bid >> 3);
    const int GM = 4;
    const int width = GM * p.tiles_n;
    const int group = swz / width;
    const int first_m = group * GM;
    const int gsize = min(p.tiles_m - first_m, GM);
    const int tm = first_m + (swz % width) % gsize;
    const int tn = (swz % width) / gsize;
    const int m0 = tm * 256, n0 = tn * 256;
    const int tid = threadIdx.x, lane = tid & 63;
    const int wave = __builtin_amdgcn_readfirstlane(tid >> 6);
    const int wm = wave >> 2, wn = wave & 3, grp = wave >> 2;
    const int g4 = lane >> 4, mm = lane & 15;

    const char* a_base = reinterpret_cast<const char*>(p.A) + (size_t)m0 * p.lda;
    const char* b_base = reinterpret_cast<const char*>(p.W) + (size_t)n0 * p.ldw;
    unsigned int a_off[4], b_off[4];
#pragma unroll
    for (int i = 0; i < 4; ++i) {
        const int row = (wave * 4 + i) * 8 + (lane >> 3);
        const int c = (lane & 7) ^ f8_swz(row);
        a_off[i] = (unsigned int)((size_t)(min(m0 + row, p.M - 1) - m0) * p.lda) + (c << 4);
        b_off[i] = (unsigned int)((size_t)(min(n0 + row, p.N - 1) - n0) * p.ldw) + (c << 4);
    }
    const int nk = p.K >> 7;
    f32x4 acc[8][4];
#pragma unroll
    for (int i = 0; i < 8; ++i)
#pragma unroll
        for (int j = 0; j < 4; ++j) acc[i][j] = (f32x4){0.f, 0.f, 0.f, 0.f};
    auto stage = [&](int buf, int kt) {
        char* base = smem + buf * STAGE;
        const char* ak = a_base + (size_t)kt * 128;
        const char* bk = b_base + (size_t)kt * 128;
#pragma unroll
        for (int i = 0; i < 4; ++i) {
            __builtin_amdgcn_global_load_lds(GLB_PTR(ak + a_off[i]), LDS_PTR(base + (wave * 4 + i) * 1024), 16, 0, 0);
            __builtin_amdgcn_global_load_lds(GLB_PTR(bk + b_off[i]), LDS_PTR(base + 32768 + (wave * 4 + i) * 1024), 16, 0, 0);
        }
    };
    const int one = 0x7f7f7f7f;
    stage(0, 0);
    asm volatile("s_waitcnt vmcnt(0)" ::: "memory");
    __builtin_amdgcn_s_barrier();
    if (grp == 1) __builtin_amdgcn_s_barrier();
    for (int kt = 0; kt < nk; ++kt) {
        const char* Ab = smem + (kt & 1) * STAGE;
        const char* Bb = Ab + 32768;
        i32x8 a[4], b[4];
        if (kt + 1 < nk) stage((kt + 1) & 1, kt + 1);
#pragma unroll
        for (int j = 0; j < 4; ++j) b[j] = lds_frag8(Bb, wn * 64 + j * 16 + mm, g4);
#pragma unroll
        for (int i = 0; i < 4; ++i) a[i] = lds_frag8(Ab, wm * 128 + i * 16 + mm, g4);
        __builtin_amdgcn_sched_barrier(0);
        __builtin_amdgcn_s_barrier();
        __builtin_amdgcn_s_setprio(1);
#pragma unroll
        for (int i = 0; i < 4; ++i)
#pragma unroll
            for (int j = 0; j < 4; ++j) acc[i][j] = __builtin_amdgcn_mfma_scale_f32_16x16x128_f8f6f4(a[i], b[j], acc[i][j], 0, 0, 0, one, 0, one);
        __builtin_amdgcn_s_setprio(0);
        __builtin_amdgcn_sched_barrier(0);
        __builtin_amdgcn_s_barrier();
#pragma unroll
        for (int i = 0; i < 4; ++i) a[i] = lds_frag8(Ab, wm * 128 + (4 + i) * 16 + mm, g4);
        asm volatile("s_waitcnt vmcnt(0)" ::: "memory");
        __builtin_amdgcn_sched_barrier(0);
        __builtin_amdgcn_s_barrier();
        __builtin_amdgcn_s_setprio(1);
#pragma unroll
        for (int i = 0; i < 4; ++i)
#pragma unroll
            for (int j = 0; j < 4; ++j) acc[4 + i][j] = __builtin_amdgcn_mfma_scale_f32_16x16x128_f8f6f4(a[i], b[j], acc[4 + i][j], 0, 0, 0, one, 0, one);
        __builtin_amdgcn_s_setprio(0);
        __builtin_amdgcn_sched_barrier(0);
        __builtin_amdgcn_s_barrier();
    }
    if (grp == 0) __builtin_amdgcn_s_barrier();

    float* Cs = reinterpret_cast<float*>(smem);
#pragma unroll
    for (int half = 0; half < 2; ++half) {
        __syncthreads();
        if (wm == half) {
#pragma unroll
            for (int i = 0; i < 8; ++i)
#pragma unroll
                for (int j = 0; j < 4; ++j)
#pragma unroll
                    for (int r = 0; r < 4; ++r) Cs[(i * 16 + 4 * g4 + r) * 256 + wn * 64 + j * 16 + mm] = acc[i][j][r];
        }
        __syncthreads();
        if (p.out_f32) epilogue_rows<bf16, float, 128, 512, 256, 2>(p, Cs, m0 + half * 128, n0, tn, tid);
        else epilogue_rows<bf16, bf16, 128, 512, 256, 2>(p, Cs, m0 + half * 128, n0, tn, tid);
    }
}

extern "C" int ullsam_gemm_fp8(const void* A8, long lda, const float* a_scale, const void* W8, long ldw, const float* w_scale, void* C,
                               long ldc, int out_f32, const float* bias, const float* residual, long ldr, int act, int M, int N, int K,
                               void* stream) {
    ULLSAM_CHECK(M > 0 && N > 0 && K > 0 && K % 128 == 0, "ullsam_gemm_fp8: K=%d must be a positive multiple of 128", K);
    ULLSAM_CHECK(((uintptr_t)A8 & 15) == 0 && ((uintptr_t)W8 & 15) == 0 && lda % 16 == 0 && ldw % 16 == 0, "ullsam_gemm_fp8: 16-byte aligned rows needed");
    ULLSAM_CHECK(a_scale && w_scale, "ullsam_gemm_fp8: scales are required");
    ULLSAM_CHECK(act >= 0 && act <= 2, "ullsam_gemm_fp8: bad act %d", act);
    GemmArgs a;
    a.A = A8; a.W = W8; a.C = C; a.bias = bias; a.residual = residual;
    a.M = M; a.N = N; a.K = K; a.lda = lda; a.ldw = ldw; a.ldc = ldc; a.ldr = ldr;
    a.res_row_mod = 0; a.act = act; a.out_f32 = out_f32;
    const int osz = out_f32 ? 4 : 2;
    bool vec = ((uintptr_t)C & 15) == 0 && (ldc * osz) % 16 == 0 && (N % 8 == 0);
    if (residual) vec = vec && ((uintptr_t)residual & 15) == 0 && (ldr % 4 == 0);
    a.group_m = 4;
    a.vec_ok = vec ? 1 : 0;
    a.ws = nullptr; a.ws_bytes = 0; a.ksplit = 1;
    a.row_scale = a_scale; a.col_scale = w_scale; a.dbg = nullptr; a.w_panels = nullptr; a.a_panels = a.out_panels = 0; a.plan = nullptr;
    a.tiles_m = (M + 255) / 256; a.tiles_n = (N + 255) / 256; a.full_tiles = a.tiles_m * a.tiles_n;
    static PerDeviceOnce attr_set;
    if (attr_set.first()) (void)hipFuncSetAttribute(reinterpret_cast<const void*>(gemm256f8_kernel), hipFuncAttributeMaxDynamicSharedMemorySize, 131072);
    gemm256f8_kernel<<<dim3(a.full_tiles), dim3(512), 131072, reinterpret_cast<hipStream_t>(stream)>>>(a);
    ULLSAM_LAUNCH_CHECK();
    return 0;
}

extern "C" int ullsam_set_gemm_tuning(int key, int value) {
    if (key == 0 && value >= 1 && value <= 1024) { g_group_m = value; return 0; }
    if (key == 1 && value >= 0 && value <= 7) { g_auto_mask = value; return 0; }
    if (key == 2 && (value == 0 || value == 2)) { g_persist = value; return 0; }
    if (key == 3 && value >= 0 && value <= 2) { g_ring_splitk = value; return 0; }
    if (key == 4 && (value == 0 || value == 1)) { g_ring_panels = value; return 0; }
    if (key == 5 && (value == 0 || value == 1)) { g_act_panels = value; return 0; }
    ullsam_set_error("ullsam_set_gemm_tuning: unknown key %d / bad value %d", key, value);
    return -1;
}
extern "C" int ullsam_set_gemm_variant(int v) {
    g_gemm_variant = v & 15; g_split_tail = (v & 64) ? 0 : 1; g_dbg = (v >> 15) & 3;
    return 0;
}

template <typename T, int EMODE = 0>
static int launch_gemm(GemmArgs a, hipStream_t stream) {
    static PerDeviceOnce attr_set;
    if (attr_set.first()) {
        (void)hipFuncSetAttribute(reinterpret_cast<const void*>(gemm128_kernel<T, EMODE>), hipFuncAttributeMaxDynamicSharedMemorySize, 65536);
    }
    const int T_ = a.tiles_m * a.tiles_n;
    const int C_ = 512;
    a.full_tiles = T_;
    a.ksplit = 1;
    const int nk = a.K / (128 / (int)sizeof(T));
    const int tail = T_ % C_;
    if (g_split_tail && a.ws && T_ > C_ && tail > 0 && tail <= C_ / 2 && nk >= 128) {
        int S = C_ / tail;
        if (S > 16) S = 16;
        if (S > nk / 4) S = nk / 4;
        if (S >= 2 && (size_t)tail * S * 65536 <= a.ws_bytes) {
            a.full_tiles = T_ - tail;
            a.ksplit = S;
        }
    }
    const int grid = a.full_tiles + (T_ - a.full_tiles) * a.ksplit;
    gemm128_kernel<T, EMODE><<<dim3(grid), dim3(256), 65536, stream>>>(a);
    ULLSAM_LAUNCH_CHECK();
    if (a.ksplit > 1) {
        gemm_tail_reduce_kernel<T, EMODE><<<dim3((T_ - a.full_tiles) * 4), dim3(256), 0, stream>>>(a);
        ULLSAM_LAUNCH_CHECK();
    }
    return 0;
}

#ifndef ULLSAM_SKINNY_NT
#define ULLSAM_SKINNY_NT 1
#endif
__device__ __forceinline__ uint4 load_w16(const bf16* ptr) {
#if ULLSAM_SKINNY_NT
    const u32x4 v = __builtin_nontemporal_load(reinterpret_cast<const u32x4*>(ptr));
    return make_uint4(v[0], v[1], v[2], v[3]);
#else
    return *reinterpret_cast<const uint4*>(ptr);
#endif
}
template <bool W8> struct SkinnyW { using elem = bf16; using vec = uint4; };
template <> struct SkinnyW<true> { using elem = unsigned char; using vec = uint2; };
__device__ __forceinline__ uint2 load_w16(const unsigned char* ptr) {
#if ULLSAM_SKINNY_NT
    const u32x2 v = __builtin_nontemporal_load(reinterpret_cast<const u32x2*>(ptr));
    return make_uint2(v[0], v[1]);
#else
    return *reinterpret_cast<const uint2*>(ptr);
#endif
}
__device__ __forceinline__ uint4 widen_w(const uint4 w) { return w; }
__device__ __forceinline__ uint4 widen_w(const uint2 w) {
    typedef __bf16 bf16x2_t __attribute__((ext_vector_type(2)));
    uint4 o;
    o.x = __builtin_bit_cast(unsigned int, (bf16x2_t)__builtin_amdgcn_cvt_scalef32_pk_bf16_fp8(w.x, 1.0f, false));
    o.y = __builtin_bit_cast(unsigned int, (bf16x2_t)__builtin_amdgcn_cvt_scalef32_pk_bf16_fp8(w.x, 1.0f, true));
    o.z = __builtin_bit_cast(unsigned int, (bf16x2_t)__builtin_amdgcn_cvt_scalef32_pk_bf16_fp8(w.y, 1.0f, false));
    o.w = __builtin_bit_cast(unsigned int, (bf16x2_t)__builtin_amdgcn_cvt_scalef32_pk_bf16_fp8(w.y, 1.0f, true));
    return o;
}

__device__ __forceinline__ void bf16x8_to_f32(const uint4 u, float (&o)[8]) {
    const unsigned int d[4] = {u.x, u.y, u.z, u.w};
#pragma unroll
    for (int j = 0; j < 4; ++j) { o[2 * j] = __uint_as_float(d[j] << 16); o[2 * j + 1] = __uint_as_float(d[j] & 0xffff0000u); }
}
__device__ __forceinline__ void dot2c(float& acc, const unsigned int a, const unsigned int b) {
    asm("v_dot2c_f32_bf16 %0, %1, %2" : "+v"(acc) : "v"(a), "v"(b));
}
__device__ __forceinline__ void dot_fence() { asm volatile("s_nop 4" ::: "memory"); }
template <int NV>
__device__ __forceinline__ float wave_sum_many(float (&v)[NV]) {
    static_assert(NV == 16 || NV == 32, "");
    const int lane = threadIdx.x & 63;
    int o = 32;
#pragma unroll
    for (int n = NV; n > 1; n >>= 1, o >>= 1) {
        const bool up = (lane & o) != 0;
#pragma unroll
        for (int i = 0; i < n / 2; ++i) {
            const float lo = v[i], hi = v[i + n / 2];
            v[i] = (up ? hi : lo) + __shfl_xor(up ? lo : hi, o, 64);
        }
    }
    float t = v[0];
#pragma unroll
    for (; o > 0; o >>= 1) t += __shfl_xor(t, o, 64);
    return t;
}

template <int MM>
struct NormRows { float4 v[MM][4]; float4 w[4]; };
template <int MM>
__device__ __forceinline__ void stage_rmsnorm_load(NormRows<MM>& n, const GemmArgs& p, const bool active = true) {
    const int tid = threadIdx.x & 255, M = active ? p.M : 0, nq = p.K >> 10;
    const long ldx = p.ldx;
    const float* xb = p.norm_x + tid * 4;
    const float* wb = p.norm_w + tid * 4;
#pragma unroll
    for (int m = 0; m < MM; ++m)
#pragma unroll
        for (int i = 0; i < 4; ++i) {
            n.v[m][i] = make_float4(0.f, 0.f, 0.f, 0.f);
            if (i < nq && m < M) n.v[m][i] = *reinterpret_cast<const float4*>(xb + m * ldx + i * 1024);
        }
#pragma unroll
    for (int i = 0; i < 4; ++i) n.w[i] = i < nq ? *reinterpret_cast<const float4*>(wb + i * 1024) : make_float4(0.f, 0.f, 0.f, 0.f);
}
template <int MM>
__device__ __forceinline__ void stage_rmsnorm_finish(const NormRows<MM>& n, char* smem, float* red, const GemmArgs& p, const bool active = true) {
    const int tid = threadIdx.x & 255, lane = tid & 63, wv = tid >> 6;
    const int K = p.K, nq = K >> 10;
    float ss[MM];
#pragma unroll
    for (int m = 0; m < MM; ++m) {
        ss[m] = 0.f;
#pragma unroll
        for (int i = 0; i < 4; ++i) ss[m] += (n.v[m][i].x * n.v[m][i].x + n.v[m][i].y * n.v[m][i].y) + (n.v[m][i].z * n.v[m][i].z + n.v[m][i].w * n.v[m][i].w);
    }
#pragma unroll
    for (int o = 32; o > 0; o >>= 1) {
        float t[MM];
#pragma unroll
        for (int m = 0; m < MM; ++m) t[m] = __shfl_xor(ss[m], o, 64);
#pragma unroll
        for (int m = 0; m < MM; ++m) ss[m] += t[m];
    }
    if (lane == 0 && active) {
#pragma unroll
        for (int m = 0; m < MM; ++m) red[wv * MM + m] = ss[m];
    }
    __syncthreads();
    bf16* dst = reinterpret_cast<bf16*>(smem) + tid * 4;
#pragma unroll
    for (int m = 0; m < MM; ++m) {
        const float tot = ((red[m] + red[MM + m]) + red[2 * MM + m]) + red[3 * MM + m];
        const float rstd = rsqrtf(tot / (float)K + p.norm_eps);
#pragma unroll
        for (int i = 0; i < 4; ++i) {
            if (i >= nq || !active) continue;
            const float4 o = make_float4(n.v[m][i].x * rstd * n.w[i].x, n.v[m][i].y * rstd * n.w[i].y, n.v[m][i].z * rstd * n.w[i].z, n.v[m][i].w * rstd * n.w[i].w);
            store4(dst + (size_t)m * K + i * 1024, o);
        }
    }
    __syncthreads();
// ... 277 lines not shown
        __shared__ float nred[16];
        stage_rmsnorm_load<4>(nrows, p);
        __builtin_amdgcn_sched_barrier(0);
        fill(b0, 0);
        __builtin_amdgcn_sched_barrier(0);
        stage_rmsnorm_finish<4>(nrows, smem, nred, p);
        fill(b1, 512 < KQ ? 512 : 0);
    } else {
        fill(b0, 0);
        if (512 < KQ) fill(b1, 512);
    }
    for (int k0 = 0; k0 < KQ; k0 += 1024) {
        step(b0, k0);
        if (k0 + 512 >= KQ) break;
        if (k0 + 1024 < KQ) fill(b0, k0 + 1024);
        step(b1, k0 + 512);
        if (k0 + 1536 < KQ) fill(b1, k0 + 1536);
    }
    dot_fence();
    {
        const float tot = wave_sum_many<R * MM>(acc);
        constexpr int SH = R * MM == 16 ? 2 : 1;
        if ((lane & ((1 << SH) - 1)) == 0) red[wv][lane >> SH] = tot;
    }
    __syncthreads();
    if (tid >= R * MM) return;
    const int r = tid / MM, m = tid - r * MM;
    if (m >= p.M) return;
    auto total = [&](const int i, const long row) {
        const float t = (red[0][i] + red[1][i]) + (red[2][i] + red[3][i]);
        if constexpr (W8) return t * p.col_scale[row]; else return t;
    };
    if (rope) {
        if (r >= 4) return;
        const long n1 = n0 + r, n2 = n1 + 64;
        const float x1 = total(r * MM + m, n1) + (p.bias ? p.bias[n1] : 0.f), x2 = total((r + 4) * MM + m, n2) + (p.bias ? p.bias[n2] : 0.f);
        const int slot = (int)(n1 >> 7), d = (int)(n1 & 127);
        const int gs = p.rope_G + 2, kv = slot / gs, g = slot - kv * gs;
        const int b = m / p.rope_S, sq = m - b * p.rope_S;
        bf16* dst;
        float o1 = x1, o2 = x2;
        if (g == gs - 1) {
            dst = reinterpret_cast<bf16*>(p.rope_v) + (((long)b * p.rope_KVH + kv) * p.rope_cap + p.rope_pos0 + sq) * 128;
        } else {
            const int ps = min(max(p.rope_pos[m], 0), p.rope_rows - 1);
            const float* cp = p.rope_cos + (size_t)ps * 128 + d;
            const float* sp = p.rope_sin + (size_t)ps * 128 + d;
            o1 = x1 * cp[0] - x2 * sp[0];
            o2 = x2 * cp[64] + x1 * sp[64];
            dst = g == gs - 2 ? reinterpret_cast<bf16*>(p.rope_k) + (((long)b * p.rope_KVH + kv) * p.rope_cap + p.rope_pos0 + sq) * 128
                              : reinterpret_cast<bf16*>(p.rope_q) + (long)m * ((long)p.rope_KVH * p.rope_G * 128) + ((long)kv * p.rope_G + g) * 128;
        }
        dst[d] = (bf16)o1;
        dst[d + 64] = (bf16)o2;
        return;
    }
    const long n = n0 + r;
    if (n >= p.N) return;
    float v = total(tid, n);
    if (p.bias) v += p.bias[n];
    if (p.act == 1) v = gelu_erf(v);
    else if (p.act == 2) v = fmaxf(v, 0.f);
    if (p.residual) v += p.residual[(size_t)(p.res_row_mod > 0 ? m % p.res_row_mod : m) * p.ldr + n];
    if (p.out_f32) reinterpret_cast<float*>(p.C)[(size_t)m * p.ldc + n] = v;
    else reinterpret_cast<bf16*>(p.C)[(size_t)m * p.ldc + n] = (bf16)v;
}

template <bool W8 = false>
static int launch_gemm_skinny(const GemmArgs& a, hipStream_t stream) {
    const bool normed = a.norm_x != nullptr;
    if (normed && (a.M > 4 || a.K > 4096 || a.K % 2048 != 0 || a.ldx % 4 != 0)) { ullsam_set_error("skinny GEMM: the fused RMSNorm prologue needs M <= 4, K <= 4096, K %% 2048 == 0 (M=%d K=%d)", a.M, a.K); return -1; }
    if (a.act == 4 && (a.M > 4 || a.K % 2048 != 0 || a.N % 128 != 0)) { ullsam_set_error("skinny GEMM: the RoPE epilogue needs M <= 4, K %% 2048 == 0 (M=%d K=%d)", a.M, a.K); return -1; }
    if (a.act == 4 || (a.act != 3 && a.N <= 8192 && a.K % 2048 == 0)) {
        const dim3 g4((unsigned)((a.N + 3) / 4)), g8((unsigned)((a.N + 7) / 8));
        const size_t lds = normed ? (size_t)4 * a.K * 2 : 0;
        if (normed) gemm_skinny_ksplit_kernel<4, 8, true, W8><<<g8, 256, lds, stream>>>(a);
        else if (a.act == 4) gemm_skinny_ksplit_kernel<4, 8, false, W8><<<g8, 256, 0, stream>>>(a);
        else if (a.M > 4) gemm_skinny_ksplit_kernel<8, 4, false, W8><<<g4, 256, 0, stream>>>(a);
        else gemm_skinny_ksplit_kernel<4, 8, false, W8><<<g8, 256, 0, stream>>>(a);
        ULLSAM_LAUNCH_CHECK();
        return 0;
    }
    const int MM = a.M <= 4 ? 4 : 8;
    const size_t lds = (size_t)MM * a.K * 2;
    const long waves = a.act == 3 ? (long)a.N / 4 : ((long)a.N + 3) / 4;
    if (MM == 4 && (normed || a.act == 3) && waves >= 4096 && lds + 256 <= 64 * 1024) {
        static PerDeviceOnce cu_once; static int n_cu = 256;
        if (cu_once.first()) { int dev = 0; hipDeviceProp_t pr; if (hipGetDevice(&dev) == hipSuccess && hipGetDeviceProperties(&pr, dev) == hipSuccess && pr.multiProcessorCount > 0) n_cu = pr.multiProcessorCount; }
        const int n_wg = n_cu * 2;
        int W = 8; double best = 1e30;
        for (int w = 8; w >= 4; --w) {
            const long per = (long)n_wg * w, trips = (waves + per - 1) / per;
            const double waste = (double)(trips * per) / (double)waves;
            if (waste < best - 1e-9) { best = waste; W = w; }
        }
        if (normed) gemm_skinny_persist_kernel<true, W8><<<n_wg, W * 64, lds, stream>>>(a, (int)waves);
        else gemm_skinny_persist_kernel<false, W8><<<n_wg, W * 64, lds, stream>>>(a, (int)waves);
        ULLSAM_LAUNCH_CHECK();
        return 0;
    }
    const dim3 grid((unsigned)((waves + 3) / 4));
    static PerDeviceOnce attr4, attr8;
    if (normed) {
        gemm_skinny_kernel<4, true, W8><<<grid, 256, lds, stream>>>(a);
    } else if (MM == 4) {
        if (attr4.first()) { (void)hipFuncSetAttribute(reinterpret_cast<const void*>(gemm_skinny_kernel<4, false, W8>), hipFuncAttributeMaxDynamicSharedMemorySize, 159 * 1024); }
        gemm_skinny_kernel<4, false, W8><<<grid, 256, lds, stream>>>(a);
    } else {
        if (attr8.first()) { (void)hipFuncSetAttribute(reinterpret_cast<const void*>(gemm_skinny_kernel<8, false, W8>), hipFuncAttributeMaxDynamicSharedMemorySize, 159 * 1024); }
        gemm_skinny_kernel<8, false, W8><<<grid, 256, lds, stream>>>(a);
    }
    ULLSAM_LAUNCH_CHECK();
    return 0;
}

struct RopeEpilogue { const int* pos; const float* cos; const float* sin; void* q; void* k; void* v; int S, KVH, G, cap, pos0, rows; };
struct NormPrologue { const float* x; long ldx; const float* w; float eps; };

static int gemm_impl(int dtype, const void* A, long lda, const void* W, long ldw, void* C, long ldc, int out_f32,
                     const float* bias, const float* residual, long ldr, int res_row_mod, int act, int M, int N,
                     int K, void* workspace, long ws_bytes, void* stream, const RopeEpilogue* rope, const NormPrologue* norm = nullptr, const void* w_panels = nullptr,
                     int a_panels = 0, int out_panels = 0, int* plan = nullptr) {
    ULLSAM_CHECK(dtype == ULLSAM_DT_F32 || dtype == ULLSAM_DT_BF16, "ullsam_gemm: bad dtype %d", dtype);
    ULLSAM_CHECK(M > 0 && N > 0 && K > 0, "ullsam_gemm: empty problem M=%d N=%d K=%d", M, N, K);
    const int esz = dtype == ULLSAM_DT_F32 ? 4 : 2;
    const int bk = 128 / esz;
    ULLSAM_CHECK(K % bk == 0, "ullsam_gemm: K=%d must be a multiple of %d", K, bk);
    ULLSAM_CHECK(((uintptr_t)A & 15) == 0 && ((uintptr_t)W & 15) == 0, "ullsam_gemm: A/W must be 16-byte aligned");
    ULLSAM_CHECK((lda * esz) % 16 == 0 && (ldw * esz) % 16 == 0, "ullsam_gemm: lda/ldw rows must be 16-byte multiples");
    const bool split_ok = (act & 256) != 0;
    act &= 255;
    ULLSAM_CHECK(act >= 0 && act <= 4 && (act == 4) == (rope != nullptr), "ullsam_gemm: bad act %d", act);
    if (act == 3) ULLSAM_CHECK(N % 128 == 0 && !bias && !residual, "ullsam_gemm: swiglu needs N%%128==0, no bias/residual");
    GemmArgs a;
    a.rope_pos = nullptr; a.rope_cos = a.rope_sin = nullptr; a.rope_q = a.rope_k = a.rope_v = nullptr;
    a.rope_S = a.rope_KVH = a.rope_G = a.rope_cap = a.rope_pos0 = a.rope_rows = 0;
    if (rope) {
        a.rope_pos = rope->pos; a.rope_cos = rope->cos; a.rope_sin = rope->sin; a.rope_q = rope->q; a.rope_k = rope->k; a.rope_v = rope->v;
        a.rope_S = rope->S; a.rope_KVH = rope->KVH; a.rope_G = rope->G; a.rope_cap = rope->cap; a.rope_pos0 = rope->pos0; a.rope_rows = rope->rows;
    }
    a.norm_x = nullptr; a.norm_w = nullptr; a.norm_eps = 0.f; a.ldx = 0;
    if (norm) {
        ULLSAM_CHECK(norm->x && norm->w && ((uintptr_t)norm->x & 15) == 0 && ((uintptr_t)norm->w & 15) == 0 && norm->ldx % 4 == 0,
                     "ullsam_gemm: the RMSNorm prologue needs 16-byte aligned fp32 rows and weight");
        a.norm_x = norm->x; a.norm_w = norm->w; a.norm_eps = norm->eps; a.ldx = norm->ldx;
    }
    ULLSAM_CHECK(!w_panels || (dtype == ULLSAM_DT_BF16 && ((uintptr_t)w_panels & 1023) == 0 && N % 16 == 0 && K % 32 == 0),
                 "ullsam_gemm: K-panels are bf16 [N / 16][K / 32][16][32], 1 KiB aligned (N=%d K=%d)", N, K);
    ULLSAM_CHECK(!a_panels || (dtype == ULLSAM_DT_BF16 && K % 32 == 0 && lda == K && ((uintptr_t)A & 1023) == 0),
                 "ullsam_gemm: activation K-panels (A) are bf16 [ceil(M / 16)][K / 32][16][32], contiguous (lda == K), 1 KiB aligned (K=%d lda=%ld)", K, lda);
    ULLSAM_CHECK(!out_panels || (dtype == ULLSAM_DT_BF16 && !out_f32 && act != 4 && (act == 3 ? N / 2 : N) % 32 == 0 && ldc == (act == 3 ? N / 2 : N) && ((uintptr_t)C & 1023) == 0),
                 "ullsam_gemm: activation K-panels (C) are bf16 [ceil(M / 16)][N_out / 32][16][32], contiguous, 1 KiB aligned (N=%d ldc=%ld)", N, ldc);
    a.A = A; a.W = W; a.C = C; a.bias = bias; a.residual = residual; a.w_panels = w_panels;
    a.a_panels = a_panels; a.out_panels = out_panels; a.plan = plan;
    auto not_ring = [&](int& rc) -> bool {
        if (plan) { plan[0] = plan[1] = 0; rc = 0; return true; }
        if (a_panels || out_panels) {
            ullsam_set_error("ullsam_gemm: activation K-panels refused: this launch (M=%d N=%d K=%d act=%d) does not reach a ring kernel -- ask the query first", M, N, K, act);
            rc = -1;
            return true;
        }
        return false;
    };
    int nr = 0;
    a.M = M; a.N = N; a.K = K;
    a.lda = lda; a.ldw = ldw; a.ldc = ldc; a.ldr = ldr;
    a.res_row_mod = res_row_mod; a.act = act; a.out_f32 = out_f32;
    const int osz = out_f32 ? 4 : esz;
    const int n_out = act == 3 ? N / 2 : N;
    bool vec = ((uintptr_t)C & 15) == 0 && (ldc * osz) % 16 == 0 && (n_out % 8 == 0);
    if (residual) vec = vec && ((uintptr_t)residual & 15) == 0 && (ldr % 4 == 0);
    a.vec_ok = vec ? 1 : 0;
    a.ws = reinterpret_cast<float*>(workspace);
    a.ws_bytes = workspace ? (size_t)ws_bytes : 0;
    a.group_m = g_group_m;
    a.row_scale = nullptr;
    a.col_scale = nullptr;
    a.dbg = (g_dbg && workspace && ws_bytes >= (56l << 20)) ? reinterpret_cast<unsigned long long*>(reinterpret_cast<char*>(workspace) + (48l << 20)) : nullptr;
    a.ksplit = 1;
    a.tiles_m = (M + 127) / 128;
    a.tiles_n = (N + 127) / 128;
    a.full_tiles = a.tiles_m * a.tiles_n;
    hipStream_t s = reinterpret_cast<hipStream_t>(stream);
    const int variant = g_gemm_variant;
    if ((variant == 0 || norm) && (act != 4 || (M <= 4 && K % 2048 == 0)) && dtype == ULLSAM_DT_BF16 && M <= 8 && K % 512 == 0 && lda % 8 == 0 && ldw % 8 == 0 &&
        (size_t)(M <= 4 ? 4 : 8) * K * 2 <= 144 * 1024 && (act != 3 || N % 128 == 0))
        return not_ring(nr) ? nr : launch_gemm_skinny<false>(a, s);
    ULLSAM_CHECK(!norm, "ullsam_gemm: the RMSNorm prologue exists in the decode-step kernels only (bf16, M <= 4, K <= 4096; got M=%d K=%d)", M, K);
    const long t256 = (long)((M + 255) / 256) * ((N + 255) / 256);
    const double fill = (double)t256 / (double)(((t256 + 255) / 256) * 256);
    const long tail256 = t256 % 256;
    const bool v3_split = g_split_tail && workspace && t256 > 256 && tail256 > 0 && tail256 <= 64 && K >= 64 * bk;
    const bool big = M >= 1024 && N >= 256 && K >= 8 * bk && (act != 3 || N % 256 == 0);
    const bool bias_v4 = !bias || (N % 4 == 0 && ((uintptr_t)bias & 15) == 0);
    const bool ring_ok = dtype == ULLSAM_DT_BF16 && act <= 3 && K % 64 == 0 && K >= 128 && bias_v4 && (act != 3 || N % 256 == 0);
    if (act == 4 && dtype == ULLSAM_DT_BF16 && M >= 1024 && K % 64 == 0 && K >= 256 && (variant == 0 || variant == 6 || variant == 9 || variant == 10) &&
        (((uintptr_t)rope->q | (uintptr_t)rope->k | (uintptr_t)rope->v) & 15) == 0 && (!bias || ((uintptr_t)bias & 15) == 0))
        return launch_gemm_ring_rope(a, s, variant == 6 ? 256 : variant == 9 ? 272 : variant == 10 ? 208 : 0);
    if (variant == 6 || variant == 8 || variant == 9) {
        if (!ring_ok || (variant == 8 && act == 3)) { ullsam_set_error("ullsam_gemm: the ring kernels need bf16, K %% 64 == 0, K >= 128, no RoPE epilogue (256x320: no SwiGLU)"); return -1; }
        return variant == 6 ? launch_gemm_v6(a, s) : variant == 8 ? launch_gemm_v8(a, s) : launch_gemm_v9(a, s);
    }
    if ((variant == 1 || variant == 3) && not_ring(nr)) return nr;
    if (variant == 1) return a.act == 4 ? (dtype == ULLSAM_DT_F32 ? launch_gemm<float, 1>(a, s) : launch_gemm<bf16, 1>(a, s))
                                        : (dtype == ULLSAM_DT_F32 ? launch_gemm<float>(a, s) : launch_gemm<bf16>(a, s));
    if (variant == 3) {
        if (act == 3 && N % 256 != 0) { ullsam_set_error("ullsam_gemm: the 256x256 kernel's SwiGLU epilogue needs N %% 256 == 0"); return -1; }
        return dtype == ULLSAM_DT_F32 ? launch_gemm_v3<float>(a, s) : launch_gemm_v3<bf16>(a, s);
    }
    if (ring_ok && variant == 0 && (g_ring_splitk == 2 || (g_ring_splitk == 1 && split_ok))) {
        int shape = 0;
        const int S = ring_splitk_plan(a, &shape);
        if (S && not_ring(nr)) return nr;
        if (S) return shape == 8 ? launch_gemm_ring_splitk<8, 8, 5>(a, S, s) : shape == 9 ? launch_gemm_ring_splitk<9, 8, 4>(a, S, s) : launch_gemm_ring_splitk<8, 8, 4>(a, S, s);
    }
    if (ring_ok && M >= 1024 && N >= 256 && K >= 256) {
        const double c256 = v3_split ? (double)(t256 / 256) + 0.5 : (double)((t256 + 255) / 256);
        const long t320 = (long)((M + 255) / 256) * (N / 320), t272 = (long)((M + 271) / 272) * ((N + 255) / 256);
        const double c320 = (N % 320 == 0 && act != 3 && (g_auto_mask & 2)) ? 1.25 * (double)((t320 + 255) / 256) : 1e9;
        const double c272 = (g_auto_mask & 4) ? 1.0625 * (double)((t272 + 255) / 256) : 1e9;
        if (c320 <= 0.96 * c256 || (act == 1 && c320 <= c256)) return launch_gemm_v8(a, s);
        if (c272 <= 0.96 * c256) return launch_gemm_v9(a, s);
        if ((g_auto_mask & 1) && big && fill >= 0.74 && !v3_split) return launch_gemm_v6(a, s);
    }
    if (not_ring(nr)) return nr;
    const bool v3 = big && (fill >= 0.74 || v3_split);
    if (v3) return dtype == ULLSAM_DT_F32 ? launch_gemm_v3<float>(a, s) : launch_gemm_v3<bf16>(a, s);
    if (a.act == 4) return dtype == ULLSAM_DT_F32 ? launch_gemm<float, 1>(a, s) : launch_gemm<bf16, 1>(a, s);
    return dtype == ULLSAM_DT_F32 ? launch_gemm<float>(a, s) : launch_gemm<bf16>(a, s);
}

extern "C" int ullsam_gemm(int dtype, const void* A, long lda, const void* W, long ldw, void* C, long ldc, int out_f32,
                           const float* bias, const float* residual, long ldr, int res_row_mod, int act, int M, int N,
                           int K, void* workspace, long ws_bytes, void* stream) {
    ULLSAM_CHECK(act != 4, "ullsam_gemm: act 4 is ullsam_gemm_qkv_rope");
    return gemm_impl(dtype, A, lda, W, ldw, C, ldc, out_f32, bias, residual, ldr, res_row_mod, act, M, N, K, workspace, ws_bytes, stream, nullptr);
}

extern "C" int ullsam_gemm_panels(int dtype, const void* A, long lda, const void* W, long ldw, const void* w_panels, void* C, long ldc, int out_f32,
                                  const float* bias, const float* residual, long ldr, int res_row_mod, int act, int M, int N,
                                  int K, void* workspace, long ws_bytes, void* stream) {
    ULLSAM_CHECK(act != 4, "ullsam_gemm_panels: act 4 is ullsam_gemm_qkv_rope_panels");
    return gemm_impl(dtype, A, lda, W, ldw, C, ldc, out_f32, bias, residual, ldr, res_row_mod, act, M, N, K, workspace, ws_bytes, stream, nullptr, nullptr, w_panels);
}

extern "C" int ullsam_gemm_rmsnorm(const float* x, long ldx, const float* norm_w, float eps, const void* W, long ldw, void* C, long ldc,
                                   int out_f32, const float* bias, const float* residual, long ldr, int act, int M, int N, int K, void* stream) {
    ULLSAM_CHECK(act != 4, "ullsam_gemm_rmsnorm: act 4 is ullsam_decode_qkv_rope");
    NormPrologue n{x, ldx, norm_w, eps};
    return gemm_impl(ULLSAM_DT_BF16, nullptr, K, W, ldw, C, ldc, out_f32, bias, residual, ldr, 0, act, M, N, K, nullptr, 0, stream, nullptr, &n);
}

extern "C" int ullsam_decode_qkv_rope(const void* a, const float* x, long ldx, const float* norm_w, float eps, const void* W, long ldw,
                                      const float* bias, int B, int K, int KVH, int G, const int* pos, const float* cos_tab,
                                      const float* sin_tab, int tab_rows, void* q_out, void* k_cache, void* v_cache, int cap, int cache_pos0,
                                      void* stream) {
    ULLSAM_CHECK(B > 0 && B <= 4 && KVH > 0 && G > 0 && tab_rows > 0 && K % 2048 == 0, "ullsam_decode_qkv_rope: B=%d (1..4) K=%d (%% 2048)", B, K);
    ULLSAM_CHECK(cache_pos0 + 1 <= cap, "ullsam_decode_qkv_rope: cache overflow (%d + 1 > %d)", cache_pos0, cap);
    RopeEpilogue r{pos, cos_tab, sin_tab, q_out, k_cache, v_cache, 1, KVH, G, cap, cache_pos0, tab_rows};
    NormPrologue n{x, ldx, norm_w, eps};
    const int N = KVH * (G + 2) * 128;
    return gemm_impl(ULLSAM_DT_BF16, norm_w ? nullptr : a, K, W, ldw, q_out, (long)KVH * G * 128, 0, bias, nullptr, 0, 0, 4, B, N, K, nullptr, 0,
                     stream, &r, norm_w ? &n : nullptr);
}

static int gemm_w8_impl(const char* who, const void* A, const NormPrologue* norm, const void* W8, long ldw, const float* w_scale, void* C, long ldc, int out_f32,
                        const float* bias, const float* residual, long ldr, int act, int M, int N, int K, void* stream, const RopeEpilogue* rope) {
    ULLSAM_CHECK(W8 && w_scale && C, "%s: null weights, scales or output", who);
    ULLSAM_CHECK(M > 0 && M <= 8 && N > 0 && K > 0 && K % 512 == 0, "%s: decode-step shapes only (1 <= M <= 8, K %% 512 == 0; got M=%d N=%d K=%d)", who, M, N, K);
    ULLSAM_CHECK((size_t)(M <= 4 ? 4 : 8) * K * 2 <= 144 * 1024, "%s: K=%d: the activation rows do not fit the LDS", who, K);
    ULLSAM_CHECK(act >= 0 && act <= 4 && (act == 4) == (rope != nullptr), "%s: bad act %d", who, act);
    ULLSAM_CHECK(((uintptr_t)W8 & 7) == 0 && ldw % 8 == 0 && ldw >= K, "%s: weight rows must be 8-byte aligned (ldw=%ld)", who, ldw);
    if (act == 3) ULLSAM_CHECK(N % 128 == 0 && !bias && !residual, "%s: swiglu needs N %% 128 == 0, no bias / residual", who);
    GemmArgs a{};
    if (rope) {
        a.rope_pos = rope->pos; a.rope_cos = rope->cos; a.rope_sin = rope->sin; a.rope_q = rope->q; a.rope_k = rope->k; a.rope_v = rope->v;
        a.rope_S = rope->S; a.rope_KVH = rope->KVH; a.rope_G = rope->G; a.rope_cap = rope->cap; a.rope_pos0 = rope->pos0; a.rope_rows = rope->rows;
    }
    if (norm) {
        ULLSAM_CHECK(norm->x && norm->w && ((uintptr_t)norm->x & 15) == 0 && ((uintptr_t)norm->w & 15) == 0 && norm->ldx % 4 == 0,
                     "%s: the RMSNorm prologue needs 16-byte aligned fp32 rows and weight", who);
        a.norm_x = norm->x; a.norm_w = norm->w; a.norm_eps = norm->eps; a.ldx = norm->ldx;
    } else {
        ULLSAM_CHECK(A && ((uintptr_t)A & 15) == 0, "%s: bf16 activations must be 16-byte aligned", who);
    }
    a.A = A; a.W = W8; a.C = C; a.bias = bias; a.residual = residual; a.col_scale = w_scale;
    a.M = M; a.N = N; a.K = K;
    a.lda = K; a.ldw = ldw; a.ldc = ldc; a.ldr = ldr;
    a.act = act; a.out_f32 = out_f32;
    a.group_m = g_group_m; a.ksplit = 1;
    return launch_gemm_skinny<true>(a, reinterpret_cast<hipStream_t>(stream));
}

extern "C" int ullsam_gemm_w8(const void* A, const float* x, long ldx, const float* norm_w, float eps, const void* W8, long ldw, const float* w_scale,
                              void* C, long ldc, int out_f32, const float* bias, const float* residual, long ldr, int act, int M, int N, int K,
                              void* stream) {
    ULLSAM_CHECK(act != 4, "ullsam_gemm_w8: act 4 is ullsam_decode_qkv_rope_w8");
    NormPrologue n{x, ldx, norm_w, eps};
    return gemm_w8_impl("ullsam_gemm_w8", norm_w ? nullptr : A, norm_w ? &n : nullptr, W8, ldw, w_scale, C, ldc, out_f32, bias, residual, ldr, act, M, N, K, stream, nullptr);
}

extern "C" int ullsam_decode_qkv_rope_w8(const void* a, const float* x, long ldx, const float* norm_w, float eps, const void* W8, long ldw,
                                         const float* w_scale, const float* bias, int B, int K, int KVH, int G, const int* pos, const float* cos_tab,
                                         const float* sin_tab, int tab_rows, void* q_out, void* k_cache, void* v_cache, int cap, int cache_pos0,
                                         void* stream) {
    ULLSAM_CHECK(B > 0 && B <= 4 && KVH > 0 && G > 0 && tab_rows > 0 && K > 0 && K % 2048 == 0, "ullsam_decode_qkv_rope_w8: B=%d (1..4) K=%d (%% 2048)", B, K);
    ULLSAM_CHECK(cache_pos0 >= 0 && cache_pos0 + 1 <= cap, "ullsam_decode_qkv_rope_w8: cache overflow (%d + 1 > %d)", cache_pos0, cap);
// ... 65 lines not shown
```

### ullsam_amd/csrc/gemm_ring8p.h

```cpp

__device__ __forceinline__ void blds16(u32x4 desc, unsigned int voff, unsigned int soff, unsigned int lds_addr) {
    unsigned int keep;
    asm volatile("s_mov_b32 %0, m0\n\ts_mov_b32 m0, %4\n\ts_nop 0\n\tbuffer_load_dwordx4 %1, %2, %3 offen lds\n\ts_mov_b32 m0, %0"
                 : "=&s"(keep) : "v"(voff), "s"(desc), "s"(soff), "s"(lds_addr) : "memory");
}
#pragma clang diagnostic push
#pragma clang diagnostic ignored "-Winline-asm"
template <int MOFF>
__device__ __forceinline__ void blds16_imm(u32x4 desc, unsigned int voff, unsigned int soff, unsigned int wave_lds_base) {
    asm volatile("s_add_i32 m0, %3, %4\n\ts_nop 0\n\tbuffer_load_dwordx4 %0, %1, %2 offen lds"
                 :: "v"(voff), "s"(desc), "s"(soff), "s"(wave_lds_base), "n"(MOFF) : "memory", "m0");
}
template <int N> __device__ __forceinline__ void wait_vmcnt() {
    static_assert(N >= 0 && N <= 6, "counted waits of the ring: one stage of a wave's pieces (at most three per operand) in flight");
    asm volatile("s_waitcnt vmcnt(%0)" :: "n"(N) : "memory");
}
#pragma clang diagnostic pop
__device__ __forceinline__ int fresh_lane() {
    int ln;
    asm volatile("v_mbcnt_lo_u32_b32 %0, -1, 0\n\tv_mbcnt_hi_u32_b32 %0, -1, %0" : "=v"(ln));
    return ln;
}
__device__ __forceinline__ u32x4 raw_desc(const void* base, unsigned int bytes) {
    const uintptr_t b = reinterpret_cast<uintptr_t>(base);
    u32x4 d;
    d[0] = __builtin_amdgcn_readfirstlane((unsigned int)b);
    d[1] = __builtin_amdgcn_readfirstlane((unsigned int)(b >> 32) & 0xffffu);
    d[2] = __builtin_amdgcn_readfirstlane(bytes);
    d[3] = 0x00020000u;
    return d;
}

template <int MI0, int MI1, int NTW, int EMODE = 0, bool STAMP = false>
__global__ __launch_bounds__(512) void gemm_ring8p_kernel(GemmArgs p) {
    extern __shared__ __attribute__((aligned(16))) char smem[];
    typedef bf16 T;
    constexpr int BM = 16 * (MI0 + MI1), BN = 64 * NTW;
    constexpr int PA = BM / 16, PB = BN / 16;
    constexpr int ASZ = BM * 64, STG = ASZ + BN * 64;
    constexpr int BIAS_LDS = 4 * STG;
    static_assert(PA >= 8 && PA <= 24 && PB >= 8 && PB <= 24, "piece assignment below: one to three pieces per wave and operand");
    static_assert(NTW == 4 || NTW == 5, "epilogue layouts below: four sub-tiles in two pairs, optionally a fifth on its own");
    constexpr int WW = 16 * NTW;

    const int nblk = p.full_tiles;
    const int q8 = nblk >> 3, r8 = nblk & 7;
    const int GMr = p.group_m;
    const int width = GMr * p.tiles_n;
    auto tile_of = [&](int v, int& tm, int& tn) __attribute__((always_inline)) {
        const int xcd = v & 7;
        const int swz = (xcd < r8 ? xcd * (q8 + 1) : r8 * (q8 + 1) + (xcd - r8) * q8) + (v >> 3);
        const int group = swz / width;
        const int first_m = group * GMr;
        const int gsize = min(p.tiles_m - first_m, GMr);
        const int rem = swz - group * width;
        tn = rem / gsize;
        tm = first_m + (rem - tn * gsize);
    };

    const int tid = threadIdx.x, lane = tid & 63;
    const int wave = __builtin_amdgcn_readfirstlane(tid >> 6);
    const int wm = wave >> 2, wn = wave & 3, grp = wave >> 2;
    const int na = (PA - wave + 7) / 8, nb = (PB - wave + 7) / 8;
    const int perm = EMODE == 1 ? 2 : p.out_f32 ? 0 : (p.act == 3 ? 2 : 1);
    auto w_row = [&](int R) {
        const int wb = R / WW, q = R - wb * WW, j = q >> 4, r = q & 15;
        if (perm == 1) return j < 4 ? WW * wb + 32 * (j >> 1) + 8 * (r >> 2) + 4 * (j & 1) + (r & 3) : WW * wb + 64 + r;
        if (perm == 2) return 128 * (wb >> 1) + 64 * (j >> 1) + 32 * (wb & 1) + 8 * (r >> 2) + 4 * (j & 1) + (r & 3);
        return R;
    };
    const bool panels = p.w_panels != nullptr;
    const int wp_shift = panels ? 4 : 0;
    const unsigned int wp_mask = panels ? 15u : 0u, wp_block = panels ? (unsigned int)p.K * 32u : (unsigned int)(p.ldw * 2);
    const unsigned int kst = __builtin_amdgcn_readfirstlane(panels ? 1024u : 64u);
    const bool a_pan = p.a_panels != 0;
    const int ap_shift = a_pan ? 4 : 0;
    const unsigned int ap_mask = a_pan ? 15u : 0u, ap_block = a_pan ? (unsigned int)p.K * 32u : (unsigned int)(p.lda * 2);
    const unsigned int akst = __builtin_amdgcn_readfirstlane(a_pan ? 1024u : 64u);
    unsigned int a_off[3], b_off[3];
    auto set_offsets = [&](int ln) __attribute__((always_inline)) {
#pragma unroll
        for (int i = 0; i < 3; ++i) {
            const int row = (wave + 8 * i) * 16 + (ln >> 2);
            const int c = (ln & 3) ^ ((row >> 2) & 2);
            a_off[i] = ((unsigned int)row >> ap_shift) * ap_block + ((unsigned int)row & ap_mask) * 64u + (c << 4);
            const unsigned int wr = (unsigned int)w_row(row);
            b_off[i] = (wr >> wp_shift) * wp_block + (wr & wp_mask) * 64u + (c << 4);
        }
    };
    set_offsets(lane);
    const u32x4 a_desc = raw_desc(p.A, a_pan ? (unsigned int)((size_t)((p.M + 15) & ~15) * p.K * 2) : (unsigned int)(((size_t)(p.M - 1) * p.lda + p.K) * 2));
    const u32x4 b_desc = raw_desc(panels ? p.w_panels : p.W, (unsigned int)(((size_t)(p.N - 1) * p.ldw + p.K) * 2));
    const unsigned int a_tile = (unsigned int)(p.lda * 2) * BM, b_tile = (unsigned int)(p.ldw * 2) * BN;
    const int st1 = p.K >> 5;
    const unsigned int wbase = __builtin_amdgcn_readfirstlane((unsigned int)(uintptr_t)LDS_PTR(smem + wave * 1024));
    const bool has_bias = p.bias && p.act != 3 && EMODE == 0;
    const int G = gridDim.x;

    auto bias_dma = [&](int n0t, int buf) __attribute__((always_inline)) {
        if (has_bias && wave < 2) {
            const int c = min(n0t + wave * 256 + fresh_lane() * 4, p.N - 4);
            glds16_sbase(reinterpret_cast<const char*>(p.bias), (unsigned int)c * 4u, (unsigned int)(uintptr_t)LDS_PTR(smem + BIAS_LDS + buf * 2048 + wave * 1024));
        }
    };
    auto request_stage = [&](unsigned int ra, unsigned int rb, int slot) __attribute__((always_inline)) {
        char* base = smem + slot * STG;
#pragma unroll
        for (int i = 0; i < 3; ++i) {
            if (i < na) blds16(a_desc, a_off[i], ra, (unsigned int)(uintptr_t)LDS_PTR(base + (wave + 8 * i) * 1024));
            if (i < nb) blds16(b_desc, b_off[i], rb, (unsigned int)(uintptr_t)LDS_PTR(base + ASZ + (wave + 8 * i) * 1024));
        }
    };
    auto stamp = [&](int tile_k, int kk) __attribute__((always_inline)) {
        if (STAMP && p.dbg && (tid & 255) == 0 && tile_k < 8) p.dbg[(((size_t)blockIdx.x * 2 + grp) * 8 + tile_k) * 4 + kk] = __builtin_amdgcn_s_memtime();
    };

    int tm0, tn0;
    tile_of(blockIdx.x, tm0, tn0);
    bias_dma(tn0 * BN, 0);
    request_stage(tm0 * a_tile, tn0 * b_tile, 0);
    request_stage(tm0 * a_tile + akst, tn0 * b_tile + kst, 1);
    asm volatile("s_waitcnt vmcnt(0)" ::: "memory");
    __builtin_amdgcn_s_barrier();
    if (grp == 1) __builtin_amdgcn_s_barrier();

    auto core = [&](auto MIW_c, auto ROWW_c) __attribute__((always_inline)) {
        constexpr int MIW = decltype(MIW_c)::value;
        constexpr int DG = 2;
        const unsigned int kstep[4] = {kst * DG, kst * (DG + 1), kst * (DG + 2), kst * (DG + 3)};
        const unsigned int akstep[4] = {akst * DG, akst * (DG + 1), akst * (DG + 2), akst * (DG + 3)};
        const int row_w = decltype(ROWW_c)::value >= 0 ? decltype(ROWW_c)::value : wm * (MI0 * 16);
        f32x4 acc[MIW][NTW];
#pragma unroll
        for (int i = 0; i < MIW; ++i)
#pragma unroll
            for (int j = 0; j < NTW; ++j) acc[i][j] = (f32x4){0.f, 0.f, 0.f, 0.f};
        unsigned int rd_a = 0, rd_b = 0;
        auto set_lane_state = [&]() __attribute__((always_inline)) {
            const int ln = fresh_lane();
            set_offsets(ln);
            const unsigned int lane_part = (unsigned int)((ln & 15) * 64 + (((ln >> 4) ^ (((ln & 15) >> 2) & 2)) << 4));
            rd_a = (unsigned int)(uintptr_t)LDS_PTR(smem) + (unsigned int)row_w * 64u + lane_part;
            rd_b = (unsigned int)(uintptr_t)LDS_PTR(smem) + (unsigned int)(ASZ + wn * (16 * NTW) * 64) + lane_part;
        };
        auto stage = [&](auto J_c, unsigned int so_a, unsigned int so_b, auto NA_c, auto NB_c) __attribute__((always_inline)) {
            constexpr int J = decltype(J_c)::value;
            constexpr int NA = decltype(NA_c)::value, NB = decltype(NB_c)::value;
            constexpr int RS = (J + DG) & 3;
            const unsigned int rq_a = so_a + akstep[J], rq_b = so_b + kstep[J];
            unsigned int t_a = rd_a, t_b = rd_b;
            if constexpr (J != 0) {
                asm volatile("v_add_u32 %0, %1, %2" : "=v"(t_a) : "n"(J * STG), "v"(rd_a));
                asm volatile("v_add_u32 %0, %1, %2" : "=v"(t_b) : "n"(J * STG), "v"(rd_b));
            }
            auto frag_at = [&](unsigned int addr) -> Frag<T> {
                Frag<T> f;
                f.v = *reinterpret_cast<const __attribute__((address_space(3))) bf16x8_t*>(addr);
                return f;
            };
            Frag<T> a8[MIW], b[NTW];
            {
                auto request = [&](auto QI_c) __attribute__((always_inline)) {
                    constexpr int qi = decltype(QI_c)::value, i = qi >> 1;
                    if constexpr (!(qi & 1) && i < NA) blds16_imm<RS * STG + i * 8192>(a_desc, a_off[i], rq_a, wbase);
                    if constexpr ((qi & 1) && i < NB) blds16_imm<RS * STG + ASZ + i * 8192>(b_desc, b_off[i], rq_b, wbase);
                    __builtin_amdgcn_sched_barrier(0);
                };
                auto rd = [&](auto R_c) __attribute__((always_inline)) {
                    constexpr int r = decltype(R_c)::value;
                    if constexpr (r < NTW + MIW) {
                        if constexpr (r < NTW) b[r] = frag_at(t_b + r * 1024);
                        else a8[r - NTW] = frag_at(t_a + (r - NTW) * 1024);
                        __builtin_amdgcn_sched_barrier(0);
                    }
                };
                request(std::integral_constant<int, 0>{});
                rd(std::integral_constant<int, 0>{}); rd(std::integral_constant<int, 1>{}); rd(std::integral_constant<int, 2>{});
                request(std::integral_constant<int, 1>{});
                rd(std::integral_constant<int, 3>{}); rd(std::integral_constant<int, 4>{}); rd(std::integral_constant<int, 5>{});
                request(std::integral_constant<int, 2>{});
                rd(std::integral_constant<int, 6>{}); rd(std::integral_constant<int, 7>{}); rd(std::integral_constant<int, 8>{});
                request(std::integral_constant<int, 3>{});
                rd(std::integral_constant<int, 9>{}); rd(std::integral_constant<int, 10>{}); rd(std::integral_constant<int, 11>{});
                request(std::integral_constant<int, 4>{});
                rd(std::integral_constant<int, 12>{}); rd(std::integral_constant<int, 13>{});
                request(std::integral_constant<int, 5>{});
            }
            wait_vmcnt<NA + NB>();
            __builtin_amdgcn_sched_barrier(0);
            __builtin_amdgcn_s_barrier();
            __builtin_amdgcn_s_setprio(1);
#pragma unroll
            for (int i = 0; i < MIW; ++i)
#pragma unroll
                for (int j = 0; j < NTW; ++j) mma16(b[j], a8[i], acc[i][j]);
            __builtin_amdgcn_s_setprio(0);
            __builtin_amdgcn_sched_barrier(0);
            __builtin_amdgcn_s_barrier();
        };
        auto run_tile = [&](auto NA_c, auto NB_c, unsigned int sa, unsigned int sb, unsigned int san, unsigned int sbn) __attribute__((always_inline)) {
            using I0 = std::integral_constant<int, 0>; using I1 = std::integral_constant<int, 1>; using I2 = std::integral_constant<int, 2>; using I3 = std::integral_constant<int, 3>;
            const int ntrip = st1 >> 2;
            const unsigned int ktrip = 4u * kst, atrip = 4u * akst;
            unsigned int ra = sa, rb = sb;
            for (int t = 0; t < ntrip; ++t) {
                const bool last = t == ntrip - 1;
                const unsigned int ha = last ? san - atrip : ra, hb = last ? sbn - ktrip : rb;
                stage(I0{}, ra, rb, NA_c, NB_c);
                stage(I1{}, ra, rb, NA_c, NB_c);
                stage(I2{}, ha, hb, NA_c, NB_c);
                stage(I3{}, ha, hb, NA_c, NB_c);
                ra += atrip; rb += ktrip;
            }
        };

        int v = blockIdx.x, tm = tm0, tn = tn0, par = 0, tile_k = 0;
        while (true) {
            stamp(tile_k, 0);
            const int vn = v + G;
            const bool has_next = vn < nblk;
            int tmn = tm, tnn = tn;
            if (has_next) tile_of(vn, tmn, tnn);
            const unsigned int sa = tm * a_tile, sb = tn * b_tile, san = tmn * a_tile, sbn = tnn * b_tile;
            {
                set_lane_state();
                constexpr int NA_LO = PA / 8, NA_HI = (PA + 7) / 8, NB_LO = PB / 8, NB_HI = (PB + 7) / 8;
                if (NA_HI != NA_LO && na == NA_HI) {
                    if (NB_HI != NB_LO && nb == NB_HI) run_tile(std::integral_constant<int, NA_HI>{}, std::integral_constant<int, NB_HI>{}, sa, sb, san, sbn);
                    else run_tile(std::integral_constant<int, NA_HI>{}, std::integral_constant<int, NB_LO>{}, sa, sb, san, sbn);
                } else {
                    if (NB_HI != NB_LO && nb == NB_HI) run_tile(std::integral_constant<int, NA_LO>{}, std::integral_constant<int, NB_HI>{}, sa, sb, san, sbn);
                    else run_tile(std::integral_constant<int, NA_LO>{}, std::integral_constant<int, NB_LO>{}, sa, sb, san, sbn);
                }
            }
            stamp(tile_k, 1);
            auto border_sync = [&](int i, int at) __attribute__((always_inline)) {
                if (i == at && grp == 0) { __builtin_amdgcn_sched_barrier(0); __builtin_amdgcn_s_barrier(); __builtin_amdgcn_sched_barrier(0); }
            };
            const int m0 = tm * BM, n0 = tn * BN;
            const int lane_e = fresh_lane();
            const int g4 = lane_e >> 4, mm = lane_e & 15;
            const char* bias_lds = smem + BIAS_LDS + par * 2048;
            float bv[4 * NTW];
#pragma unroll
            for (int e = 0; e < 4 * NTW; ++e) bv[e] = 0.f;
            if (has_bias) {
#pragma unroll
                for (int t = 0; t < NTW; ++t) {
                    const int col = wn * WW + ((p.out_f32 || t == 4) ? 16 * t + 4 * g4 : 32 * (t >> 1) + 8 * g4 + 4 * (t & 1));
                    const float4 x = *reinterpret_cast<const float4*>(bias_lds + col * 4);
                    bv[4 * t] = x.x; bv[4 * t + 1] = x.y; bv[4 * t + 2] = x.z; bv[4 * t + 3] = x.w;
                }
            }
            {
                const bool odd = mm & 1;
                const int row0 = m0 + row_w + mm;
                const int rowp = row0 & ~1;
                auto gst = [&](void* ptr, u32x4 vv) __attribute__((always_inline)) { *reinterpret_cast<u32x4*>(ptr) = vv; };
                const bool o_pan = p.out_panels != 0;
                const size_t o_cells = (size_t)((p.act == 3 ? p.N >> 1 : p.N) >> 5);
                const size_t o_r16 = o_pan ? o_cells * 512 : (size_t)16 * p.ldc, o_r1 = o_pan ? (size_t)32 : (size_t)p.ldc;
                auto o_at = [&](int row, int col) __attribute__((always_inline)) -> size_t {
                    return o_pan ? ((size_t)(row >> 4) * o_cells + (size_t)(col >> 5)) * 512 + (size_t)((row & 15) * 32 + (col & 31)) : (size_t)row * p.ldc + col;
                };
                if constexpr (EMODE == 1) {
                    const int slot = (n0 >> 7) + (wn >> 1), d = 32 * (wn & 1) + 8 * g4;
                    const int gs = p.rope_G + 2, kv = slot / gs, g = slot - kv * gs;
                    const bool live = slot < p.rope_KVH * gs;
                    const bool rotate = g != gs - 1;
                    float bl[8], bh[8];
    #pragma unroll
                    for (int e = 0; e < 8; ++e) { bl[e] = (p.bias && live) ? p.bias[slot * 128 + d + e] : 0.f; bh[e] = (p.bias && live) ? p.bias[slot * 128 + d + 64 + e] : 0.f; }
                    T* const Q = reinterpret_cast<T*>(p.rope_q);
                    T* const KVc = reinterpret_cast<T*>(g == gs - 2 ? p.rope_k : p.rope_v);
                    int ps[MIW];
    #pragma unroll
                    for (int i = 0; i < MIW; ++i) {
                        const int gm = row0 + 16 * i;
                        ps[i] = (live && rotate && gm < p.M) ? min(max(p.rope_pos[gm], 0), p.rope_rows - 1) : 0;
                    }
                    float4 cn[2], sn[2];
                    auto load_cs = [&](int i, float4 (&c)[2], float4 (&s_)[2]) __attribute__((always_inline)) {
                        const float* cp = p.rope_cos + (size_t)ps[i] * 128 + d;
                        const float* sp = p.rope_sin + (size_t)ps[i] * 128 + d;
                        c[0] = *reinterpret_cast<const float4*>(cp); c[1] = *reinterpret_cast<const float4*>(cp + 4);
                        s_[0] = *reinterpret_cast<const float4*>(sp); s_[1] = *reinterpret_cast<const float4*>(sp + 4);
                    };
                    if (rotate) load_cs(0, cn, sn);
    #pragma unroll
                    for (int i = 0; i < MIW; ++i) {
                        border_sync(i, 1);
                        const float4 c0 = cn[0], c1 = cn[1], s0 = sn[0], s1 = sn[1];
                        if (rotate && i + 1 < MIW) load_cs(i + 1, cn, sn);
                        const int gm = row0 + 16 * i;
                        if (gm >= p.M || !live) continue;
                        float x[8], y[8], lo[8], hi[8];
    #pragma unroll
                        for (int e = 0; e < 8; ++e) { x[e] = acc[i][e >> 2][e & 3] + bl[e]; y[e] = acc[i][2 + (e >> 2)][e & 3] + bh[e]; }
                        if (rotate) {
                            const float cv[8] = {c0.x, c0.y, c0.z, c0.w, c1.x, c1.y, c1.z, c1.w}, sv[8] = {s0.x, s0.y, s0.z, s0.w, s1.x, s1.y, s1.z, s1.w};
    #pragma unroll
                            for (int e = 0; e < 8; ++e) { lo[e] = fmaf(x[e], cv[e], -(y[e] * sv[e])); hi[e] = fmaf(y[e], cv[e], x[e] * sv[e]); }
                        } else {
    #pragma unroll
                            for (int e = 0; e < 8; ++e) { lo[e] = x[e]; hi[e] = y[e]; }
                        }
                        T* dst;
                        if (g < p.rope_G) dst = Q + (size_t)gm * ((size_t)p.rope_KVH * p.rope_G * 128) + (size_t)(kv * p.rope_G + g) * 128 + d;
                        else {
                            const int bi = gm / p.rope_S, sq = gm - bi * p.rope_S;
                            dst = KVc + (((size_t)bi * p.rope_KVH + kv) * p.rope_cap + p.rope_pos0 + sq) * 128 + d;
                        }
                        gst(dst, (u32x4){pack_bf16x2(lo[0], lo[1]), pack_bf16x2(lo[2], lo[3]), pack_bf16x2(lo[4], lo[5]), pack_bf16x2(lo[6], lo[7])});
                        gst(dst + 64, (u32x4){pack_bf16x2(hi[0], hi[1]), pack_bf16x2(hi[2], hi[3]), pack_bf16x2(hi[4], hi[5]), pack_bf16x2(hi[6], hi[7])});
                    }
                } else if (!p.out_f32 && p.act != 3) {
                    const int colb = n0 + wn * WW + (odd ? 32 : 0) + 8 * g4;
                    T* cp = reinterpret_cast<T*>(p.C) + o_at(rowp, colb);
                    const int col5 = n0 + wn * WW + 64 + 4 * g4;
                    T* cp5 = reinterpret_cast<T*>(p.C) + o_at(row0, col5);
                    auto drain = [&](auto ACT) __attribute__((always_inline)) {
                        uint2 w5 = make_uint2(0u, 0u);
                        auto actf = [&](float x) __attribute__((always_inline)) {
                            if constexpr (decltype(ACT)::value == 1) return gelu_erfc5(x);
                            else if constexpr (decltype(ACT)::value == 2) return fmaxf(x, 0.f);
                            else return x;
                        };
    #pragma unroll
                        for (int i = 0; i < MIW; ++i) {
                            border_sync(i, 1);
                            unsigned int o[8];
    #pragma unroll
                            for (int h = 0; h < 2; ++h)
    #pragma unroll
                                for (int q = 0; q < 4; ++q)
                                    o[4 * h + q] = pack_bf16x2(actf(acc[i][2 * h + (q >> 1)][2 * (q & 1)] + bv[8 * h + 2 * q]),
                                                               actf(acc[i][2 * h + (q >> 1)][2 * (q & 1) + 1] + bv[8 * h + 2 * q + 1]));
                            u32x4 s0, s1;
                            pair_swap((u32x4){o[0], o[1], o[2], o[3]}, (u32x4){o[4], o[5], o[6], o[7]}, odd, s0, s1);
                            if (rowp + 16 * i < p.M) {
                                gst(cp + i * o_r16, s0);
                                gst(cp + i * o_r16 + o_r1, s1);
                            }
                            if constexpr (NTW == 5) {
                                uint2 w;
                                w.x = pack_bf16x2(actf(acc[i][4][0] + bv[16]), actf(acc[i][4][1] + bv[17]));
                                w.y = pack_bf16x2(actf(acc[i][4][2] + bv[18]), actf(acc[i][4][3] + bv[19]));
                                if constexpr (MIW % 2 == 0) {
                                    if (i & 1) {
                                        const auto rx = __builtin_amdgcn_permlane16_swap(w5.x, w.x, false, false);
                                        const auto ry = __builtin_amdgcn_permlane16_swap(w5.y, w.y, false, false);
                                        const int r5 = row0 + 16 * (i - 1 + (g4 & 1));
                                        if (r5 < p.M)
                                            gst(reinterpret_cast<T*>(p.C) + o_at(r5, n0 + wn * WW + 64 + 8 * (g4 >> 1)), (u32x4){rx[0], ry[0], rx[1], ry[1]});
                                    } else {
                                        w5 = w;
                                    }
                                } else {
                                    if (row0 + 16 * i < p.M) *reinterpret_cast<uint2*>(cp5 + i * o_r16) = w;
                                }
                            }
                        }
                    };
                    if (p.act == 1) drain(std::integral_constant<int, 1>{});
                    else if (p.act == 2) drain(std::integral_constant<int, 2>{});
                    else drain(std::integral_constant<int, 0>{});
                } else if (NTW == 4 && !p.out_f32 && p.act == 3) {
                    T* cp = reinterpret_cast<T*>(p.C) + o_at(row0, (n0 >> 1) + (wn >> 1) * 64 + (wn & 1) * 32 + 8 * g4);
    #pragma unroll
                    for (int i = 0; i < MIW; ++i) {
                        border_sync(i, 1);
                        unsigned int o[4];
    #pragma unroll
                        for (int q = 0; q < 4; ++q) {
                            const float g0 = acc[i][q >> 1][2 * (q & 1)], g1 = acc[i][q >> 1][2 * (q & 1) + 1];
                            const float u0 = acc[i][2 + (q >> 1)][2 * (q & 1)], u1 = acc[i][2 + (q >> 1)][2 * (q & 1) + 1];
                            o[q] = pack_bf16x2(g0 * __builtin_amdgcn_rcpf(1.0f + __expf(-g0)) * u0, g1 * __builtin_amdgcn_rcpf(1.0f + __expf(-g1)) * u1);
                        }
                        if (row0 + 16 * i < p.M) gst(cp + i * o_r16, (u32x4){o[0], o[1], o[2], o[3]});
                    }
                } else {
                    const int colp = n0 + wn * WW + (odd ? 16 : 0) + 4 * g4;
                    float* cp = reinterpret_cast<float*>(p.C) + (size_t)rowp * p.ldc + colp;
                    const int col5 = n0 + wn * WW + 64 + 4 * g4;
                    float* cp5 = reinterpret_cast<float*>(p.C) + (size_t)row0 * p.ldc + col5;
                    auto load_res = [&](int i, float4 (&r)[5]) __attribute__((always_inline)) {
    #pragma unroll
                        for (int rsel = 0; rsel < 2; ++rsel) {
                            const int gm = min(rowp + 16 * i + rsel, p.M - 1);
                            const int rr = p.res_row_mod > 0 ? gm % p.res_row_mod : gm;
                            const float* rp = p.residual + (size_t)rr * p.ldr + colp;
    #pragma unroll
                            for (int jp = 0; jp < 2; ++jp) r[2 * jp + rsel] = *reinterpret_cast<const float4*>(rp + 32 * jp);
                        }
                        if constexpr (NTW == 5) {
                            const int gm = min(row0 + 16 * i, p.M - 1);
                            const int rr = p.res_row_mod > 0 ? gm % p.res_row_mod : gm;
                            r[4] = *reinterpret_cast<const float4*>(p.residual + (size_t)rr * p.ldr + col5);
                        }
                    };
                    auto put = [&](int i, const float4 (&r)[5]) __attribute__((always_inline)) {
    #pragma unroll
                        for (int jp = 0; jp < 2; ++jp) {
                            u32x4 lo, hi, s0, s1;
    #pragma unroll
                            for (int e = 0; e < 4; ++e) {
                                lo[e] = __float_as_uint(acc[i][2 * jp][e] + bv[8 * jp + e]);
                                hi[e] = __float_as_uint(acc[i][2 * jp + 1][e] + bv[8 * jp + 4 + e]);
                            }
                            pair_swap(lo, hi, odd, s0, s1);
                            const float4 r0 = r[2 * jp], r1 = r[2 * jp + 1];
                            s0 = (u32x4){__float_as_uint(__uint_as_float(s0[0]) + r0.x), __float_as_uint(__uint_as_float(s0[1]) + r0.y),
                                         __float_as_uint(__uint_as_float(s0[2]) + r0.z), __float_as_uint(__uint_as_float(s0[3]) + r0.w)};
                            s1 = (u32x4){__float_as_uint(__uint_as_float(s1[0]) + r1.x), __float_as_uint(__uint_as_float(s1[1]) + r1.y),
                                         __float_as_uint(__uint_as_float(s1[2]) + r1.z), __float_as_uint(__uint_as_float(s1[3]) + r1.w)};
                            if (rowp + 16 * i < p.M) {
                                *reinterpret_cast<u32x4*>(cp + (size_t)(16 * i) * p.ldc + 32 * jp) = s0;
                                *reinterpret_cast<u32x4*>(cp + (size_t)(16 * i + 1) * p.ldc + 32 * jp) = s1;
                            }
                        }
                        if constexpr (NTW == 5) {
                            if (row0 + 16 * i < p.M)
                                *reinterpret_cast<float4*>(cp5 + (size_t)(16 * i) * p.ldc) = make_float4(acc[i][4][0] + bv[16] + r[4].x, acc[i][4][1] + bv[17] + r[4].y,
                                                                                                         acc[i][4][2] + bv[18] + r[4].z, acc[i][4][3] + bv[19] + r[4].w);
                        }
                    };
                    auto drain = [&](auto RES) __attribute__((always_inline)) {
                        float4 ra[5], rb[5];
    #pragma unroll
                        for (int j = 0; j < 5; ++j) ra[j] = rb[j] = make_float4(0.f, 0.f, 0.f, 0.f);
                        if constexpr (decltype(RES)::value) load_res(0, ra);
    #pragma unroll
                        for (int i = 0; i < MIW; i += 2) {
                            border_sync(i, 2);
                            if constexpr (decltype(RES)::value) { if (i + 1 < MIW) load_res(i + 1, rb); __builtin_amdgcn_sched_barrier(0); }
                            put(i, ra);
                            if constexpr (decltype(RES)::value) { if (i + 2 < MIW) load_res(i + 2, ra); __builtin_amdgcn_sched_barrier(0); }
                            if (i + 1 < MIW) put(i + 1, rb);
                        }
                    };
                    if (p.residual) drain(std::true_type{}); else drain(std::false_type{});
                }
            }
            stamp(tile_k, 2);
            if (has_next) bias_dma(tnn * BN, par ^ 1);
            asm volatile("s_waitcnt vmcnt(0)" ::: "memory");
            __builtin_amdgcn_s_waitcnt(0x0F70);
            stamp(tile_k, 3);
            if (grp == 1) __builtin_amdgcn_s_barrier();
            if (!has_next) break;
#pragma unroll
            for (int i = 0; i < MIW; ++i)
#pragma unroll
                for (int j = 0; j < NTW; ++j) acc[i][j] = (f32x4){0.f, 0.f, 0.f, 0.f};
            v = vn; tm = tmn; tn = tnn;
            par ^= 1; ++tile_k;
        }
    };
    if constexpr (MI0 == MI1) core(std::integral_constant<int, MI0>{}, std::integral_constant<int, -1>{});
    else {
        if (wm == 0) core(std::integral_constant<int, MI0>{}, std::integral_constant<int, 0>{});
        else core(std::integral_constant<int, MI1>{}, std::integral_constant<int, MI0 * 16>{});
    }
    if (grp == 0) __builtin_amdgcn_s_barrier();
}

template <int MI0, int MI1, int NTW, int EMODE = 0>
static int launch_gemm_ring8p(GemmArgs a, hipStream_t stream, int max_wgs) {
    constexpr int BM = 16 * (MI0 + MI1), BN = 64 * NTW;
    constexpr int LDS = 4 * (BM + BN) * 64 + 4096;
    static_assert(LDS <= 163840, "160 KiB of LDS per CU");
    static PerDeviceOnce attr_set;
    if (attr_set.first()) {
        (void)hipFuncSetAttribute(reinterpret_cast<const void*>(gemm_ring8p_kernel<MI0, MI1, NTW, EMODE, false>), hipFuncAttributeMaxDynamicSharedMemorySize, LDS);
        (void)hipFuncSetAttribute(reinterpret_cast<const void*>(gemm_ring8p_kernel<MI0, MI1, NTW, EMODE, true>), hipFuncAttributeMaxDynamicSharedMemorySize, LDS);
    }
    a.tiles_m = (a.M + BM - 1) / BM;
    a.tiles_n = a.N / BN;
    a.full_tiles = a.tiles_m * a.tiles_n;
    a.ksplit = 1;
    const int grid = a.full_tiles < max_wgs ? a.full_tiles : max_wgs;
    if (a.dbg) gemm_ring8p_kernel<MI0, MI1, NTW, EMODE, true><<<dim3(grid), dim3(512), LDS, stream>>>(a);
    else gemm_ring8p_kernel<MI0, MI1, NTW, EMODE, false><<<dim3(grid), dim3(512), LDS, stream>>>(a);
    ULLSAM_LAUNCH_CHECK();
    return 0;
}
```

Before: 57.50 images/s.

## Permute fp32 epilogue columns and prefetch residual rows earlier in ring GEMM

Adds a column permutation (perm 3) for NTW=5 fp32-output tiles so each wave's stores land on aligned cache lines. For NTW=4 fp32 residual epilogues it adds a three-deep residual prefetch (drain3) and issues the first residual load during the last K stage. The aim is to hide residual-read latency and cut partial-line writes in the epilogue. The cost is more register pressure from the rs[3][5] buffers, plus added complexity in bias indexing and the permuted columns.

```diff
diff --git a/include/ullsam_hip.h b/include/ullsam_hip.h
--- a/include/ullsam_hip.h
+++ b/include/ullsam_hip.h
@@ -18,6 +18,7 @@
 int ullsam_device_count(void);
 int ullsam_set_gemm_variant(int variant);
 int ullsam_set_gemm_tuning(int key, int value);
+int ullsam_ring_out_col(int ntw, int perm, int R);
 int ullsam_set_attn_variant(int variant);
 int ullsam_set_attn_debug(void* stamps);
 
diff --git a/ullsam_amd/_lib.py b/ullsam_amd/_lib.py
--- a/ullsam_amd/_lib.py
+++ b/ullsam_amd/_lib.py
@@ -170,7 +170,7 @@
     "ullsam_decode_qkv_rope_w8": [vp, vp, i64, vp, f32, vp, i64, vp, vp, i32, i32, i32, i32, vp, vp, vp, i32, vp, vp, vp, i32, i32, vp],
 }
 PLAIN = {"ullsam_last_error_string": ([], C.c_char_p), "ullsam_abi_version": ([], i32), "ullsam_device_count": ([], i32),
-         "ullsam_set_gemm_variant": ([i32], i32), "ullsam_set_gemm_tuning": ([i32, i32], i32), "ullsam_set_attn_variant": ([i32], i32),
+         "ullsam_set_gemm_variant": ([i32], i32), "ullsam_set_gemm_tuning": ([i32, i32], i32), "ullsam_ring_out_col": ([i32, i32, i32], i32),"ullsam_set_attn_variant": ([i32], i32),
          "ullsam_set_norm_variant": ([i32], i32), "ullsam_train_set_matmul_mfma": ([i32], i32), "ullsam_train_set_matmul_vec": ([i32], i32), "ullsam_train_set_rows_reg": ([i32], i32), "ullsam_set_skinny_linear_mfma": ([i32], i32), "ullsam_set_attn_debug": ([vp], i32)}
 
 
diff --git a/ullsam_amd/csrc/gemm.hip b/ullsam_amd/csrc/gemm.hip
--- a/ullsam_amd/csrc/gemm.hip
+++ b/ullsam_amd/csrc/gemm.hip
@@ -1,4 +1,5 @@
 #include "common.h"
+#include <cstdlib>
 #include <type_traits>
 
 struct GemmArgs {
@@ -27,6 +28,7 @@
     int group_m;
     int a_panels, out_panels;
     int* plan;
+    int epi;
 };
 
 #ifndef ULLSAM_RING_ASM_DMA
@@ -37,6 +39,8 @@
 static int g_gemm_variant = 0;
 static int g_dbg = 0;
 static int g_auto_mask = 7;
+static int g_fp32_epi = [] { const char* e = getenv("ULLSAM_FP32_EPILOGUE"); return (e && e[0] == '0' && !e[1]) ? 0 : 1; }();
+static int g_fp32_epi_parts = 3;
 static int g_group_m = 4;
 
 template <typename T>
@@ -648,6 +652,17 @@
                  : "=&s"(keep) : "v"(off), "s"(base), "s"(lds_addr) : "memory");
 }
 
+__host__ __device__ constexpr int ring_out_col(int ntw, int perm, int R) {
+    const int WW = 16 * ntw, wb = R / WW, q = R - wb * WW, j = q >> 4, r = q & 15;
+    if (perm == 1) return j < 4 ? WW * wb + 32 * (j >> 1) + 8 * (r >> 2) + 4 * (j & 1) + (r & 3) : WW * wb + 64 + r;
+    if (perm == 2) return 128 * (wb >> 1) + 64 * (j >> 1) + 32 * (wb & 1) + 8 * (r >> 2) + 4 * (j & 1) + (r & 3);
+    if (perm == 3 && ntw == 5) return j < 4 ? 32 * (5 * (wb >> 1) + 3 * (wb & 1) + (j >> 1)) + 16 * (j & 1) + r : 32 * (5 * (wb >> 1) + 2) + 16 * (wb & 1) + r;
+    return R;
+}
+__host__ __device__ constexpr int ring_f32_col0(int ntw, int perm, int wn) { return ring_out_col(ntw, perm, 16 * ntw * wn); }
+__host__ __device__ constexpr int ring_f32_col5(int ntw, int perm, int wn) { return ring_out_col(ntw, perm, 16 * ntw * wn + 64); }
+static_assert(ring_out_col(5, 3, 80) == 96 && ring_out_col(5, 3, 80 + 79) == 95 && ring_out_col(5, 3, 319) == 255 && ring_out_col(5, 3, 240) == 256, "perm 3: waves 1 and 3 start on lines L3 and L8");
+
 template <int MI0, int MI1, int NTW, bool STAMP = false, int EMODE = 0>
 __global__ __launch_bounds__(512) void gemm_ring8_kernel(GemmArgs p) {
     extern __shared__ __attribute__((aligned(16))) char smem[];
@@ -691,13 +706,9 @@
     const int na = (PA - wave + 7) / 8, nb = (PB - wave + 7) / 8;
     static_assert(NTW == 4 || NTW == 5, "epilogue layouts below: four sub-tiles in two pairs, optionally a fifth on its own");
     constexpr int WW = 16 * NTW;
-    const int perm = EMODE == 1 ? 2 : p.out_f32 ? 0 : (p.act == 3 ? 2 : 1);
-    auto w_row = [&](int R) {
-        const int wb = R / WW, q = R - wb * WW, j = q >> 4, r = q & 15;
-        if (perm == 1) return j < 4 ? WW * wb + 32 * (j >> 1) + 8 * (r >> 2) + 4 * (j & 1) + (r & 3) : WW * wb + 64 + r;
-        if (perm == 2) return 128 * (wb >> 1) + 64 * (j >> 1) + 32 * (wb & 1) + 8 * (r >> 2) + 4 * (j & 1) + (r & 3);
-        return R;
-    };
+    const int perm = EMODE == 1 ? 2 : p.out_f32 ? ((NTW == 5 && (p.epi & 1)) ? 3 : 0) : (p.act == 3 ? 2 : 1);
+    auto w_row = [&](int R) { return ring_out_col(NTW, perm, R); };
+    const int fc0 = ring_f32_col0(NTW, perm, wn), fc5 = ring_f32_col5(NTW, perm, wn);
     unsigned int a_off[3], b_off[3];
 #pragma unroll
     for (int i = 0; i < 3; ++i) {
@@ -753,6 +764,27 @@
             __builtin_amdgcn_global_load_lds(GLB_PTR(p.bias + c), LDS_PTR(bias_lds + wave * 1024), 16, 0, 0);
         }
     };
+    const bool direct = p.vec_ok && (p.N & 7) == 0 && (p.M & 1) == 0 && (p.out_f32 || !p.residual);
+    auto load_res = [&](int i, float4 (&r)[5]) __attribute__((always_inline)) {
+        const int row0 = m0 + row_w + mm, rowp = row0 & ~1;
+        const int colp = n0 + fc0 + ((mm & 1) ? 16 : 0) + 4 * g4, col5 = n0 + fc5 + 4 * g4;
+#pragma unroll
+        for (int rsel = 0; rsel < 2; ++rsel) {
+            const int gm = min(rowp + 16 * i + rsel, p.M - 1);
+            const int rr = p.res_row_mod > 0 ? gm % p.res_row_mod : gm;
+            const float* rp = p.residual + (size_t)rr * p.ldr + colp;
+#pragma unroll
+            for (int jp = 0; jp < 2; ++jp) r[2 * jp + rsel] = colp + 32 * jp < p.N ? *reinterpret_cast<const float4*>(rp + 32 * jp) : make_float4(0.f, 0.f, 0.f, 0.f);
+        }
+        if constexpr (NTW == 5) {
+            const int gm = min(row0 + 16 * i, p.M - 1);
+            const int rr = p.res_row_mod > 0 ? gm % p.res_row_mod : gm;
+            r[4] = col5 < p.N ? *reinterpret_cast<const float4*>(p.residual + (size_t)rr * p.ldr + col5) : make_float4(0.f, 0.f, 0.f, 0.f);
+        }
+    };
+    constexpr bool RES_EARLY = EMODE == 0 && NTW == 4;
+    const bool res_early = RES_EARLY && (p.epi & 2) && direct && p.out_f32 && p.act == 0 && p.residual;
+    float4 rs[3][5];
     stage(0);
     if (1 < st1) { stage(1); wait_one_left(); }
     else asm volatile("s_waitcnt vmcnt(0)" ::: "memory");
@@ -764,11 +796,14 @@
     auto stamp16 = [&](int kk) {
         if (STAMP && p.dbg && (tid & 255) == 0) p.dbg[(1 << 19) + ((size_t)bid * 2 + grp) * 8 + kk] = __builtin_amdgcn_s_memtime();
     };
+    auto stampw = [&](int kk) {
+        if (STAMP && p.dbg && lane == 0 && bid < (1 << 14)) p.dbg[(1 << 18) + ((size_t)bid * 8 + wave) * 2 + kk] = __builtin_amdgcn_s_memtime();
+    };
     stamp(0);
     {
-        auto body = [&](int s, auto NA_c, auto NB_c, auto MORE_c) __attribute__((always_inline)) {
+        auto body = [&](int s, auto NA_c, auto NB_c, auto MORE_c, auto LAST_c) __attribute__((always_inline)) {
             constexpr int NA = decltype(NA_c)::value, NB = decltype(NB_c)::value;
-            constexpr bool MORE = decltype(MORE_c)::value;
+            constexpr bool MORE = decltype(MORE_c)::value, LAST = decltype(LAST_c)::value;
             const char* Ab = smem + (s & 3) * STG;
             const char* Bb = Ab + ASZ;
             Frag<T> a8[MI], b[NTW];
@@ -806,6 +841,9 @@
             else if constexpr (NA + NB == 3) asm volatile("s_waitcnt vmcnt(3)" ::: "memory");
             else asm volatile("s_waitcnt vmcnt(2)" ::: "memory");
             __builtin_amdgcn_sched_barrier(0);
+            if constexpr (LAST) {
+                if (res_early) { load_res(0, rs[0]); __builtin_amdgcn_sched_barrier(0); }
+            }
             __builtin_amdgcn_s_barrier();
             __builtin_amdgcn_s_setprio(1);
 #pragma unroll
@@ -820,9 +858,14 @@
         };
         auto run = [&](auto NA_c, auto NB_c) __attribute__((always_inline)) {
             int s = 0;
-            for (; s + 2 < st1; ++s) body(s, NA_c, NB_c, std::true_type{});
+            for (; s + 2 < st1; ++s) body(s, NA_c, NB_c, std::true_type{}, std::false_type{});
             bias_dma();
-            for (; s < st1; ++s) body(s, NA_c, NB_c, std::false_type{});
+            if constexpr (RES_EARLY) {
+                if (s + 1 < st1) { body(s, NA_c, NB_c, std::false_type{}, std::false_type{}); ++s; }
+                body(s, NA_c, NB_c, std::false_type{}, std::true_type{});
+            } else {
+                for (; s < st1; ++s) body(s, NA_c, NB_c, std::false_type{}, std::false_type{});
+            }
         };
         constexpr int NA_LO = PA / 8, NA_HI = (PA + 7) / 8, NB_LO = PB / 8, NB_HI = (PB + 7) / 8;
         if (NA_HI != NA_LO && na == NA_HI) {
@@ -835,13 +878,14 @@
     }
     if (grp == 0) __builtin_amdgcn_s_barrier();
     stamp(1);
+    stampw(0);
     float bv[4 * NTW];
 #pragma unroll
     for (int e = 0; e < 4 * NTW; ++e) bv[e] = 0.f;
     if (has_bias) {
 #pragma unroll
         for (int t = 0; t < NTW; ++t) {
-            const int col = wn * WW + ((p.out_f32 || t == 4) ? 16 * t + 4 * g4 : 32 * (t >> 1) + 8 * g4 + 4 * (t & 1));
+            const int col = p.out_f32 ? (t == 4 ? fc5 : fc0 + 16 * t) + 4 * g4 : wn * WW + (t == 4 ? 16 * t + 4 * g4 : 32 * (t >> 1) + 8 * g4 + 4 * (t & 1));
             const float4 x = *reinterpret_cast<const float4*>(bias_lds + col * 4);
             bv[4 * t] = x.x; bv[4 * t + 1] = x.y; bv[4 * t + 2] = x.z; bv[4 * t + 3] = x.w;
         }
@@ -851,7 +895,6 @@
         const bool odd = mm & 1;
         const int row0 = m0 + row_w + mm;
         const int rowp = row0 & ~1;
-        const bool direct = p.vec_ok && (p.N & 7) == 0 && (p.M & 1) == 0 && (p.out_f32 || !p.residual);
         auto gst = [&](void* ptr, u32x4 v) __attribute__((always_inline)) { *reinterpret_cast<u32x4*>(ptr) = v; };
         const bool o_pan = p.out_panels != 0;
         const size_t o_cells = (size_t)((p.act == 3 ? p.N >> 1 : p.N) >> 5);
@@ -975,25 +1018,10 @@
                 if (row0 + 16 * i < p.M) gst(cp + i * o_r16, (u32x4){o[0], o[1], o[2], o[3]});
             }
         } else if (direct && p.out_f32 && p.act == 0) {
-            const int colp = n0 + wn * WW + (odd ? 16 : 0) + 4 * g4;
+            const int colp = n0 + fc0 + (odd ? 16 : 0) + 4 * g4;
             float* cp = reinterpret_cast<float*>(p.C) + (size_t)rowp * p.ldc + colp;
-            const int col5 = n0 + wn * WW + 64 + 4 * g4;
+            const int col5 = n0 + fc5 + 4 * g4;
             float* cp5 = reinterpret_cast<float*>(p.C) + (size_t)row0 * p.ldc + col5;
-            auto load_res = [&](int i, float4 (&r)[5]) __attribute__((always_inline)) {
-#pragma unroll
-                for (int rsel = 0; rsel < 2; ++rsel) {
-                    const int gm = min(rowp + 16 * i + rsel, p.M - 1);
-                    const int rr = p.res_row_mod > 0 ? gm % p.res_row_mod : gm;
-                    const float* rp = p.residual + (size_t)rr * p.ldr + colp;
-#pragma unroll
-                    for (int jp = 0; jp < 2; ++jp) r[2 * jp + rsel] = colp + 32 * jp < p.N ? *reinterpret_cast<const float4*>(rp + 32 * jp) : make_float4(0.f, 0.f, 0.f, 0.f);
-                }
-                if constexpr (NTW == 5) {
-                    const int gm = min(row0 + 16 * i, p.M - 1);
-                    const int rr = p.res_row_mod > 0 ? gm % p.res_row_mod : gm;
-                    r[4] = col5 < p.N ? *reinterpret_cast<const float4*>(p.residual + (size_t)rr * p.ldr + col5) : make_float4(0.f, 0.f, 0.f, 0.f);
-                }
-            };
             auto put = [&](int i, const float4 (&r)[5]) __attribute__((always_inline)) {
 #pragma unroll
                 for (int jp = 0; jp < 2; ++jp) {
@@ -1033,13 +1061,24 @@
                     if (i + 1 < MI && (i + 1 < MI1 || i + 1 < mi)) put(i + 1, rb);
                 }
             };
-            if (p.residual) drain(std::true_type{}); else drain(std::false_type{});
+            auto drain3 = [&]() __attribute__((always_inline)) {
+                if (!res_early) load_res(0, rs[0]);
+                if (1 < MI) load_res(1, rs[1]);
+#pragma unroll
+                for (int i = 0; i < MI; ++i) {
+                    if (i + 2 < MI) load_res(i + 2, rs[(i + 2) % 3]);
+                    __builtin_amdgcn_sched_barrier(0);
+                    if (i < MI1 || i < mi) put(i, rs[i % 3]);
+                }
+            };
+            if (EMODE == 0 && NTW == 4 && p.residual && (p.epi & 2)) drain3();
+            else if (p.residual) drain(std::true_type{}); else drain(std::false_type{});
         } else {
             float* Cs = reinterpret_cast<float*>(smem);
             auto ncol = [&](int j) __attribute__((always_inline)) {
                 if (perm == 1) return j < 4 ? WW * wn + 32 * (j >> 1) + 8 * g4 + 4 * (j & 1) : WW * wn + 64 + 4 * g4;
                 if (perm == 2) return 128 * (wn >> 1) + 64 * (j >> 1) + 32 * (wn & 1) + 8 * g4 + 4 * (j & 1);
-                return WW * wn + 16 * j + 4 * g4;
+                return (j < 4 ? fc0 + 16 * j : fc5) + 4 * g4;
             };
             auto staged = [&](auto half_c) __attribute__((always_inline)) {
                 constexpr int half = decltype(half_c)::value;
@@ -1062,6 +1101,7 @@
         }
     }
     stamp(2);
+    stampw(1);
     if (STAMP && p.dbg && (tid & 255) == 0) p.dbg[((size_t)bid * 2 + grp) * 4 + 3] = t_entry;
 }
 
@@ -1121,6 +1161,7 @@
     if (attr_set.first()) (void)hipFuncSetAttribute(reinterpret_cast<const void*>(gemm_ring8_kernel<MI0, MI1, NTW, false, 2>), hipFuncAttributeMaxDynamicSharedMemorySize, LDS);
     GemmArgs b = a;
     b.C = a.ws; b.ldc = a.N; b.out_f32 = 1; b.bias = nullptr; b.residual = nullptr; b.act = 0; b.vec_ok = 1; b.dbg = nullptr; b.w_panels = nullptr; b.a_panels = b.out_panels = 0;
+    b.epi = g_fp32_epi ? g_fp32_epi_parts : 0;
     b.tiles_m = (a.M + BM - 1) / BM;
     b.tiles_n = (a.N + BN - 1) / BN;
     b.full_tiles = b.tiles_m * b.tiles_n;
@@ -1171,6 +1212,7 @@
 template <int MI0, int MI1, int NTW, int EMODE = 0>
 static int launch_ring(const GemmArgs& a0, hipStream_t stream) {
     GemmArgs a = a0;
+    a.epi = g_fp32_epi ? g_fp32_epi_parts : 0;
     if (!(g_ring_panels && a.N % (64 * NTW) == 0 && a.K % 32 == 0 && a.ldw == a.K)) a.w_panels = nullptr;
     const int n_out = a.act == 3 ? a.N / 2 : a.N;
     const bool a_ok = g_act_panels && EMODE != 2 && a.K % 32 == 0 && a.lda == a.K && ((uintptr_t)a.A & 1023) == 0;
@@ -1326,7 +1368,7 @@
     a.group_m = 4;
     a.vec_ok = vec ? 1 : 0;
     a.ws = nullptr; a.ws_bytes = 0; a.ksplit = 1;
-    a.row_scale = a_scale; a.col_scale = w_scale; a.dbg = nullptr; a.w_panels = nullptr; a.a_panels = a.out_panels = 0; a.plan = nullptr;
+    a.row_scale = a_scale; a.col_scale = w_scale; a.dbg = nullptr; a.w_panels = nullptr; a.a_panels = a.out_panels = 0; a.plan = nullptr; a.epi = 0;
     a.tiles_m = (M + 255) / 256; a.tiles_n = (N + 255) / 256; a.full_tiles = a.tiles_m * a.tiles_n;
     static PerDeviceOnce attr_set;
     if (attr_set.first()) (void)hipFuncSetAttribute(reinterpret_cast<const void*>(gemm256f8_kernel), hipFuncAttributeMaxDynamicSharedMemorySize, 131072);
@@ -1342,8 +1384,14 @@
     if (key == 3 && value >= 0 && value <= 2) { g_ring_splitk = value; return 0; }
     if (key == 4 && (value == 0 || value == 1)) { g_ring_panels = value; return 0; }
     if (key == 5 && (value == 0 || value == 1)) { g_act_panels = value; return 0; }
+    if (key == 6 && (value == 0 || value == 1)) { g_fp32_epi = value; return 0; }
+    if (key == 7 && value >= 0 && value <= 3) { g_fp32_epi_parts = value; return 0; }
     ullsam_set_error("ullsam_set_gemm_tuning: unknown key %d / bad value %d", key, value);
     return -1;
+}
+extern "C" int ullsam_ring_out_col(int ntw, int perm, int R) {
+    if ((ntw != 4 && ntw != 5) || perm < 0 || perm > 3 || R < 0 || R >= 64 * ntw || (perm == 2 && ntw != 4) || (perm == 3 && ntw != 5)) return -1;
+    return ring_out_col(ntw, perm, R);
 }
 extern "C" int ullsam_set_gemm_variant(int v) {
     g_gemm_variant = v & 15; g_split_tail = (v & 64) ? 0 : 1; g_dbg = (v >> 15) & 3;
@@ -1927,7 +1975,7 @@
     ULLSAM_CHECK(!out_panels || (dtype == ULLSAM_DT_BF16 && !out_f32 && act != 4 && (act == 3 ? N / 2 : N) % 32 == 0 && ldc == (act == 3 ? N / 2 : N) && ((uintptr_t)C & 1023) == 0),
                  "ullsam_gemm: activation K-panels (C) are bf16 [ceil(M / 16)][N_out / 32][16][32], contiguous, 1 KiB aligned (N=%d ldc=%ld)", N, ldc);
     a.A = A; a.W = W; a.C = C; a.bias = bias; a.residual = residual; a.w_panels = w_panels;
-    a.a_panels = a_panels; a.out_panels = out_panels; a.plan = plan;
+    a.a_panels = a_panels; a.out_panels = out_panels; a.plan = plan; a.epi = 0;
     auto not_ring = [&](int& rc) -> bool {
         if (plan) { plan[0] = plan[1] = 0; rc = 0; return true; }
         if (a_panels || out_panels) {
diff --git a/ullsam_amd/csrc/gemm_ring8p.h b/ullsam_amd/csrc/gemm_ring8p.h
--- a/ullsam_amd/csrc/gemm_ring8p.h
+++ b/ullsam_amd/csrc/gemm_ring8p.h
@@ -62,13 +62,8 @@
     const int wave = __builtin_amdgcn_readfirstlane(tid >> 6);
     const int wm = wave >> 2, wn = wave & 3, grp = wave >> 2;
     const int na = (PA - wave + 7) / 8, nb = (PB - wave + 7) / 8;
-    const int perm = EMODE == 1 ? 2 : p.out_f32 ? 0 : (p.act == 3 ? 2 : 1);
-    auto w_row = [&](int R) {
-        const int wb = R / WW, q = R - wb * WW, j = q >> 4, r = q & 15;
-        if (perm == 1) return j < 4 ? WW * wb + 32 * (j >> 1) + 8 * (r >> 2) + 4 * (j & 1) + (r & 3) : WW * wb + 64 + r;
-        if (perm == 2) return 128 * (wb >> 1) + 64 * (j >> 1) + 32 * (wb & 1) + 8 * (r >> 2) + 4 * (j & 1) + (r & 3);
-        return R;
-    };
+    const int perm = EMODE == 1 ? 2 : p.out_f32 ? ((NTW == 5 && (p.epi & 1)) ? 3 : 0) : (p.act == 3 ? 2 : 1);
+    auto w_row = [&](int R) { return ring_out_col(NTW, perm, R); };
     const bool panels = p.w_panels != nullptr;
     const int wp_shift = panels ? 4 : 0;
     const unsigned int wp_mask = panels ? 15u : 0u, wp_block = panels ? (unsigned int)p.K * 32u : (unsigned int)(p.ldw * 2);
@@ -247,7 +242,8 @@
             if (has_bias) {
 #pragma unroll
                 for (int t = 0; t < NTW; ++t) {
-                    const int col = wn * WW + ((p.out_f32 || t == 4) ? 16 * t + 4 * g4 : 32 * (t >> 1) + 8 * g4 + 4 * (t & 1));
+                    const int col = p.out_f32 ? (t == 4 ? ring_f32_col5(NTW, perm, wn) : ring_f32_col0(NTW, perm, wn) + 16 * t) + 4 * g4
+                                              : wn * WW + (t == 4 ? 16 * t + 4 * g4 : 32 * (t >> 1) + 8 * g4 + 4 * (t & 1));
                     const float4 x = *reinterpret_cast<const float4*>(bias_lds + col * 4);
                     bv[4 * t] = x.x; bv[4 * t + 1] = x.y; bv[4 * t + 2] = x.z; bv[4 * t + 3] = x.w;
                 }
@@ -380,9 +376,9 @@
                         if (row0 + 16 * i < p.M) gst(cp + i * o_r16, (u32x4){o[0], o[1], o[2], o[3]});
                     }
                 } else {
-                    const int colp = n0 + wn * WW + (odd ? 16 : 0) + 4 * g4;
+                    const int colp = n0 + ring_f32_col0(NTW, perm, wn) + (odd ? 16 : 0) + 4 * g4;
                     float* cp = reinterpret_cast<float*>(p.C) + (size_t)rowp * p.ldc + colp;
-                    const int col5 = n0 + wn * WW + 64 + 4 * g4;
+                    const int col5 = n0 + ring_f32_col5(NTW, perm, wn) + 4 * g4;
                     float* cp5 = reinterpret_cast<float*>(p.C) + (size_t)row0 * p.ldc + col5;
                     auto load_res = [&](int i, float4 (&r)[5]) __attribute__((always_inline)) {
     #pragma unroll
@@ -439,7 +435,20 @@
                             if (i + 1 < MIW) put(i + 1, rb);
                         }
                     };
-                    if (p.residual) drain(std::true_type{}); else drain(std::false_type{});
+                    auto drain3 = [&]() __attribute__((always_inline)) {
+                        float4 rs[3][5];
+                        load_res(0, rs[0]);
+                        load_res(1, rs[1]);
+    #pragma unroll
+                        for (int i = 0; i < MIW; ++i) {
+                            border_sync(i, 2);
+                            if (i + 2 < MIW) load_res(i + 2, rs[(i + 2) % 3]);
+                            __builtin_amdgcn_sched_barrier(0);
+                            put(i, rs[i % 3]);
+                        }
+                    };
+                    if (NTW == 4 && p.residual && (p.epi & 2)) drain3();
+                    else if (p.residual) drain(std::true_type{}); else drain(std::false_type{});
                 }
             }
             stamp(tile_k, 2);
```

Result: slower. 54.61 images/s (-5.0%).
